# GlaireDaggers/Pretty-Fast-Video

Measured on AMD Instinct MI355X. Metric: macroblocks/s (encode+decode) 1080p YUV420, higher is better.
Workload: dtype i32 (encoder transforms evaluated in exact f32; decoders i32)

## Files before the change

include/pfv_hip_ext.h:

```cpp
#ifndef PFV_HIP_EXT_H
#define PFV_HIP_EXT_H

#include "pfv_hip_core.h"

#ifdef __cplusplus
extern "C" {
#endif

PFV_API int pfv_ctx_create_prio(int device, int priority, pfv_ctx **out);
PFV_API int pfv_ctx_pci_bus_id(pfv_ctx *ctx, char *out, int len);
PFV_API int pfv_device_sync(pfv_ctx *ctx);
PFV_API void *pfv_ctx_stream(pfv_ctx *ctx);

typedef enum pfv_option {
    PFV_OPT_ENC_TRANSFORM = 1, PFV_OPT_TILE_COMPACTION = 2, PFV_OPT_LANE_MAPPING = 3, PFV_OPT_ENTROPY_DECODE = 4,
    PFV_OPT_ENTDEC_LANE_BITS = 5, PFV_OPT_ENTDEC_LAUNCHES = 6, PFV_OPT_ENTDEC_INNER_ROUNDS = 7
} pfv_option;
enum { PFV_ENTROPY_DECODE_AUTO = 0, PFV_ENTROPY_DECODE_HOST = 1, PFV_ENTROPY_DECODE_DEVICE = 2 };
enum { PFV_LANES_AUTO = 0, PFV_LANES_PER_MB_8 = 1, PFV_LANES_PER_MB_16 = 2 };
enum { PFV_ENC_TRANSFORM_AUTO = 0, PFV_ENC_TRANSFORM_INT = 1 };
PFV_API int pfv_ctx_set_option(pfv_ctx *ctx, int option, int value);
PFV_API int pfv_ctx_get_option(pfv_ctx *ctx, int option, int *value);

typedef struct pfv_event pfv_event;
PFV_API int pfv_event_create(pfv_ctx *ctx, pfv_event **out);
PFV_API int pfv_event_record(pfv_event *e);
PFV_API int pfv_event_elapsed_ms(pfv_event *start, pfv_event *stop, float *ms);
PFV_API void pfv_event_destroy(pfv_event *e);
PFV_API int pfv_ctx_wait_event(pfv_ctx *ctx, pfv_event *e);

typedef struct pfv_graph pfv_graph;
PFV_API int pfv_graph_begin(pfv_ctx *ctx);
PFV_API int pfv_graph_end(pfv_ctx *ctx, pfv_graph **out);
PFV_API int pfv_graph_launch(pfv_graph *g);
PFV_API void pfv_graph_destroy(pfv_graph *g);

PFV_API int pfv_blit_dev(pfv_ctx *ctx, uint8_t *dst, int dst_w, int dst_h, const uint8_t *src, int src_w, int src_h,
                         int dx, int dy, int sx, int sy, int sw, int sh);

PFV_API int pfv_reduce_dev(pfv_ctx *ctx, uint8_t *dst, const uint8_t *src, int src_w, int src_h);
PFV_API int pfv_double_dev(pfv_ctx *ctx, uint8_t *dst, const uint8_t *src, int src_w, int src_h);
PFV_API int pfv_rgb_to_yuv420_dev(pfv_ctx *ctx, const uint8_t *rgb_dev, int width, int height, uint8_t *frame_dev);
PFV_API int pfv_yuv420_to_rgb_dev(pfv_ctx *ctx, const uint8_t *frame_dev, int width, int height, uint8_t *rgb_dev);

typedef struct pfv_comm pfv_comm;
enum { PFV_COMM_SUM = 0, PFV_COMM_MAX = 1 };
PFV_API int pfv_comm_unique_id(uint8_t id_out[128]);
PFV_API int pfv_comm_init(pfv_ctx *ctx, int rank, int world, const uint8_t id[128], pfv_comm **out);
PFV_API int pfv_comm_rank(const pfv_comm *c);
PFV_API int pfv_comm_world(const pfv_comm *c);
PFV_API int pfv_comm_broadcast_dev(pfv_comm *c, void *buf_dev, size_t bytes, int root);
PFV_API int pfv_comm_allreduce_f64_dev(pfv_comm *c, double *buf_dev, size_t count, int op);
PFV_API int pfv_comm_allgather_dev(pfv_comm *c, const void *send_dev, void *recv_dev, size_t bytes_per_rank);
PFV_API int pfv_comm_allreduce_f64(pfv_comm *c, double *values, size_t count, int op);
PFV_API int pfv_comm_barrier(pfv_comm *c);
PFV_API void pfv_comm_destroy(pfv_comm *c);

PFV_API int pfv_synth_frames_dev(pfv_ctx *ctx, int width, int height, int n_streams, const uint64_t *seeds, int t,
                                 uint8_t *frames_dev);
enum { PFV_SYNTH_PAN = 0, PFV_SYNTH_LOW_MOTION = 1, PFV_SYNTH_STATIC = 2 };
PFV_API int pfv_synth_frames_kind_dev(pfv_ctx *ctx, int width, int height, int n_streams, const uint64_t *seeds, int t, int kind,
                                      uint8_t *frames_dev);

PFV_API int pfv_dev_alloc(pfv_ctx *ctx, size_t bytes, void **out);
PFV_API int pfv_dev_free(pfv_ctx *ctx, void *p);
PFV_API int pfv_dev_copy(pfv_ctx *ctx, void *dst_dev, const void *src_dev, size_t bytes);
PFV_API int pfv_host_alloc(pfv_ctx *ctx, size_t bytes, void **out);
PFV_API int pfv_host_free(pfv_ctx *ctx, void *p);
PFV_API int pfv_dev_upload(pfv_ctx *ctx, void *dst_dev, const void *src_host, size_t bytes);
// ... 145 lines not shown
```

pretty-fast-video_amd/_lib.py:

```python
from __future__ import annotations

import ctypes
import os
from ctypes import POINTER, c_char_p, c_float, c_int, c_size_t, c_uint8, c_void_p

_HERE = os.path.dirname(os.path.abspath(__file__))
DEFAULT_LIB = os.path.join(_HERE, "libpfv_hip.so")

PFV_OK = 0
PFV_ERR_BAD_ARG = -1
PFV_ERR_HIP = -2
PFV_ERR_NOMEM = -3
PFV_ERR_BAD_MV = -4
PFV_ERR_NO_DEVICE = -5
PFV_ERR_FORMAT = -6
PFV_ERR_VERSION = -7
PFV_ERR_IO = -8
PFV_ERR_STATE = -9

PFV_COMM_SUM, PFV_COMM_MAX = 0, 1
PFV_OPT_ENC_TRANSFORM = 1
PFV_OPT_TILE_COMPACTION = 2
PFV_OPT_LANE_MAPPING = 3
PFV_LANES_AUTO, PFV_LANES_PER_MB_8, PFV_LANES_PER_MB_16 = 0, 1, 2
PFV_OPT_ENTROPY_DECODE = 4
PFV_OPT_ENTDEC_LANE_BITS, PFV_OPT_ENTDEC_LAUNCHES, PFV_OPT_ENTDEC_INNER_ROUNDS = 5, 6, 7
PFV_ENTROPY_DECODE_AUTO, PFV_ENTROPY_DECODE_HOST, PFV_ENTROPY_DECODE_DEVICE = 0, 1, 2
PFV_ENC_TRANSFORM_AUTO, PFV_ENC_TRANSFORM_INT = 0, 1
PFV_FRAME_PACKED, PFV_FRAME_PADDED = 0, 1


class PfvError(RuntimeError):
    def __init__(self, code: int, msg: str):
        super().__init__(f"pfv_hip error {code}: {msg}")
        self.code = code


_P = c_void_p
SIGNATURES = [
    ("pfv_device_count", c_int, []),
    ("pfv_ctx_create", c_int, [c_int, POINTER(_P)]),
    ("pfv_ctx_create_prio", c_int, [c_int, c_int, POINTER(_P)]),
    ("pfv_ctx_destroy", None, [_P]),
    ("pfv_ctx_pci_bus_id", c_int, [_P, _P, c_int]),
    ("pfv_ctx_sync", c_int, [_P]),
    ("pfv_device_sync", c_int, [_P]),
    ("pfv_ctx_stream", _P, [_P]),
    ("pfv_last_error", c_char_p, [_P]),
    ("pfv_version", c_char_p, []),
    ("pfv_ctx_set_option", c_int, [_P, c_int, c_int]),
    ("pfv_ctx_get_option", c_int, [_P, c_int, POINTER(c_int)]),
    ("pfv_event_create", c_int, [_P, POINTER(_P)]),
    ("pfv_event_record", c_int, [_P]),
    ("pfv_event_elapsed_ms", c_int, [_P, _P, POINTER(c_float)]),
    ("pfv_event_destroy", None, [_P]),
    ("pfv_ctx_wait_event", c_int, [_P, _P]),
    ("pfv_graph_begin", c_int, [_P]),
    ("pfv_graph_end", c_int, [_P, POINTER(_P)]),
    ("pfv_graph_launch", c_int, [_P]),
    ("pfv_graph_destroy", None, [_P]),
    ("pfv_pad16", c_int, [c_int]),
    ("pfv_qtables_from_quality", c_int, [c_int, _P, _P, _P, _P, POINTER(c_float)]),
    ("pfv_encode_plane", c_int, [_P, _P, c_int, c_int, _P, c_uint8, _P]),
    ("pfv_encode_plane_delta", c_int, [_P, _P, c_int, c_int, _P, _P, c_float, c_uint8, _P, _P, _P]),
    ("pfv_decode_plane_into", c_int, [_P, _P, c_int, c_int, _P, _P]),
    ("pfv_decode_plane_delta", c_int, [_P, _P, _P, _P, c_int, c_int, _P, _P, _P]),
    ("pfv_decode_plane_delta_into", c_int, [_P, _P, _P, _P, c_int, c_int, _P, _P]),
    ("pfv_blit_dev", c_int, [_P, _P, c_int, c_int, _P, c_int, c_int, c_int, c_int, c_int, c_int, c_int, c_int]),
    ("pfv_reduce_dev", c_int, [_P, _P, _P, c_int, c_int]),
    ("pfv_double_dev", c_int, [_P, _P, _P, c_int, c_int]),
    ("pfv_rgb_to_yuv420_dev", c_int, [_P, _P, c_int, c_int, _P]),
    ("pfv_yuv420_to_rgb_dev", c_int, [_P, _P, c_int, c_int, _P]),
    ("pfv_comm_unique_id", c_int, [_P]),
    ("pfv_comm_init", c_int, [_P, c_int, c_int, _P, POINTER(_P)]),
    ("pfv_comm_rank", c_int, [_P]),
    ("pfv_comm_world", c_int, [_P]),
    ("pfv_comm_broadcast_dev", c_int, [_P, _P, c_size_t, c_int]),
    ("pfv_comm_allreduce_f64_dev", c_int, [_P, _P, c_size_t, c_int]),
    ("pfv_comm_allgather_dev", c_int, [_P, _P, _P, c_size_t]),
# ... 172 lines not shown
```

pretty-fast-video_amd/csrc/pfv_context.hip:

```cpp
struct pfv_ctx {
    int device = 0;
    hipStream_t stream = nullptr;
    std::string err;
    void *scratch[8] = {};
    size_t scratch_cap[8] = {};
    QTab *qtab_dev = nullptr;
    QTab *qtab_host = nullptr;
    int *flag_dev = nullptr;
    int n_cus = 256;
    bool capturing = false;
    int opt_enc_transform = PFV_ENC_TRANSFORM_AUTO;
    int opt_tile_compaction = 1;
    int opt_lane_mapping = PFV_LANES_AUTO;
    int opt_entropy_decode = PFV_ENTROPY_DECODE_AUTO;
    int opt_entdec_lane_bits = (int)kEdSubBits, opt_entdec_launches = 3, opt_entdec_inner = kEdInner;
    std::vector<struct pfv_comm *> comms;
    std::mutex comms_m;
    pfv_ctx *owner = nullptr;
    std::vector<pfv_ctx *> children;
    int priority = 0;
};
static int ctx_create_child(pfv_ctx *user, pfv_ctx **out)
{
    int rc = pfv_ctx_create_prio(user->device, user->priority, out);
    if (rc) return rc;
    (*out)->owner = user;
    std::lock_guard<std::mutex> lk(user->comms_m);
    user->children.push_back(*out);
    return PFV_OK;
}
static void comm_teardown(struct pfv_comm *c);

static thread_local std::string g_tls_err;

static int fail(pfv_ctx *ctx, int code, const std::string &msg)
{
    if (ctx) ctx->err = msg;
    if (ctx && ctx->owner) ctx->owner->err = msg;
    g_tls_err = msg;
    return code;
}
static int hip_fail(pfv_ctx *ctx, hipError_t e, const char *what)
{
    (void)hipGetLastError();
    return fail(ctx, e == hipErrorOutOfMemory ? PFV_ERR_NOMEM : PFV_ERR_HIP,
                std::string(what) + ": " + hipGetErrorString(e));
}
#define HIP_TRY(ctx, expr)                                        \
    do {                                                          \
        hipError_t e__ = (expr);                                  \
        if (e__ != hipSuccess) return hip_fail(ctx, e__, #expr);  \
    } while (0)

static inline int pad16(int x) { return x + (16 - (x % 16)) % 16; }

extern "C" {

#ifndef PFV_BUILD_ID
#define PFV_BUILD_ID "unstamped"
#endif
PFV_API const char *pfv_version(void) { return "pfv-hip 0.2 (gfx950; pfv-rs 0.2.2 / codec 2.1.1 hot path; src " PFV_BUILD_ID ")"; }
PFV_API int pfv_pad16(int x) { return pad16(x); }

PFV_API const char *pfv_last_error(pfv_ctx *ctx) { return ctx ? ctx->err.c_str() : g_tls_err.c_str(); }

PFV_API int pfv_ctx_set_option(pfv_ctx *ctx, int option, int value)
{
    if (!ctx) return fail(nullptr, PFV_ERR_BAD_ARG, "null ctx");
    switch (option) {
    case PFV_OPT_ENC_TRANSFORM:
        if (value != PFV_ENC_TRANSFORM_AUTO && value != PFV_ENC_TRANSFORM_INT) return fail(ctx, PFV_ERR_BAD_ARG, "PFV_OPT_ENC_TRANSFORM: unknown value");
        ctx->opt_enc_transform = value;
        return PFV_OK;
    case PFV_OPT_TILE_COMPACTION:
        if (value < 0 || value > 2) return fail(ctx, PFV_ERR_BAD_ARG, "PFV_OPT_TILE_COMPACTION: 0, 1 or 2");
        ctx->opt_tile_compaction = value;
        return PFV_OK;
    case PFV_OPT_LANE_MAPPING:
        if (value != PFV_LANES_AUTO && value != PFV_LANES_PER_MB_8 && value != PFV_LANES_PER_MB_16) return fail(ctx, PFV_ERR_BAD_ARG, "PFV_OPT_LANE_MAPPING: unknown value");
        ctx->opt_lane_mapping = value;
        return PFV_OK;
    case PFV_OPT_ENTROPY_DECODE:
        if (value != PFV_ENTROPY_DECODE_AUTO && value != PFV_ENTROPY_DECODE_HOST && value != PFV_ENTROPY_DECODE_DEVICE) return fail(ctx, PFV_ERR_BAD_ARG, "PFV_OPT_ENTROPY_DECODE: unknown value");
        ctx->opt_entropy_decode = value;
        return PFV_OK;
    case PFV_OPT_ENTDEC_LANE_BITS:
        if (value < 32 || value > (int)kEdMaxSubBits || value % 32) return fail(ctx, PFV_ERR_BAD_ARG, "PFV_OPT_ENTDEC_LANE_BITS: a multiple of 32 in 32..256");
        ctx->opt_entdec_lane_bits = value;
        return PFV_OK;
    case PFV_OPT_ENTDEC_LAUNCHES:
        if (value < 1 || value > 64) return fail(ctx, PFV_ERR_BAD_ARG, "PFV_OPT_ENTDEC_LAUNCHES: 1..64");
        ctx->opt_entdec_launches = value;
        return PFV_OK;
    case PFV_OPT_ENTDEC_INNER_ROUNDS:
        if (value < 1 || value > 1024) return fail(ctx, PFV_ERR_BAD_ARG, "PFV_OPT_ENTDEC_INNER_ROUNDS: 1..1024");
        ctx->opt_entdec_inner = value;
        return PFV_OK;
    default:
        return fail(ctx, PFV_ERR_BAD_ARG, "pfv_ctx_set_option: unknown option");
    }
}
PFV_API int pfv_ctx_get_option(pfv_ctx *ctx, int option, int *value)
{
    if (!ctx || !value) return fail(ctx, PFV_ERR_BAD_ARG, "pfv_ctx_get_option: bad argument");
    switch (option) {
    case PFV_OPT_ENC_TRANSFORM: *value = ctx->opt_enc_transform; return PFV_OK;
    case PFV_OPT_TILE_COMPACTION: *value = ctx->opt_tile_compaction; return PFV_OK;
    case PFV_OPT_LANE_MAPPING: *value = ctx->opt_lane_mapping; return PFV_OK;
    case PFV_OPT_ENTROPY_DECODE: *value = ctx->opt_entropy_decode; return PFV_OK;
    case PFV_OPT_ENTDEC_LANE_BITS: *value = ctx->opt_entdec_lane_bits; return PFV_OK;
    case PFV_OPT_ENTDEC_LAUNCHES: *value = ctx->opt_entdec_launches; return PFV_OK;
    case PFV_OPT_ENTDEC_INNER_ROUNDS: *value = ctx->opt_entdec_inner; return PFV_OK;
    default: return fail(ctx, PFV_ERR_BAD_ARG, "pfv_ctx_get_option: unknown option");
    }
}

PFV_API int pfv_device_count(void)
{
    int n = 0;
    if (hipGetDeviceCount(&n) != hipSuccess) { (void)hipGetLastError(); return 0; }
    return n;
}

PFV_API int pfv_ctx_create(int device, pfv_ctx **out) { return pfv_ctx_create_prio(device, 0, out); }

PFV_API int pfv_ctx_create_prio(int device, int priority, pfv_ctx **out)
{
    if (!out) return fail(nullptr, PFV_ERR_BAD_ARG, "pfv_ctx_create: out is null");
    *out = nullptr;
    int n = 0;
    hipError_t e = hipGetDeviceCount(&n);
    if (e != hipSuccess || n <= 0) {
        (void)hipGetLastError();
        return fail(nullptr, PFV_ERR_NO_DEVICE, "pfv_ctx_create: no HIP device visible (the HIP path has no CPU fallback)");
    }
    if (device < 0 || device >= n) return fail(nullptr, PFV_ERR_BAD_ARG, "pfv_ctx_create: device ordinal out of range");
    HIP_TRY(nullptr, hipSetDevice(device));
    pfv_ctx *ctx = new pfv_ctx();
    ctx->device = device;
    ctx->priority = priority;
    {
        int cus = 0;
        if (hipDeviceGetAttribute(&cus, hipDeviceAttributeMultiprocessorCount, device) == hipSuccess && cus > 0) ctx->n_cus = cus;
    }
    if (priority == 0) {
        e = hipStreamCreateWithFlags(&ctx->stream, hipStreamNonBlocking);
    } else {
        int least = 0, greatest = 0;
        e = hipDeviceGetStreamPriorityRange(&least, &greatest);
        if (e == hipSuccess) e = hipStreamCreateWithPriority(&ctx->stream, hipStreamNonBlocking, priority > 0 ? greatest : least);
    }
    if (e == hipSuccess) e = hipMalloc((void **)&ctx->qtab_dev, 4 * sizeof(QTab));
    if (e == hipSuccess) e = hipHostMalloc((void **)&ctx->qtab_host, 4 * sizeof(QTab), hipHostMallocDefault);
    if (e == hipSuccess) e = hipMalloc((void **)&ctx->flag_dev, sizeof(int));
    if (e == hipSuccess) e = hipMemsetAsync(ctx->flag_dev, 0, sizeof(int), ctx->stream);
    if (e != hipSuccess) {
        int rc = hip_fail(nullptr, e, "pfv_ctx_create");
        pfv_ctx_destroy(ctx);
        return rc;
    }
    *out = ctx;
    return PFV_OK;
}

PFV_API void pfv_ctx_destroy(pfv_ctx *ctx)
// ... 160 lines not shown
```

pretty-fast-video_amd/csrc/pfv_device.h:

```cpp
#pragma once
#include <stdint.h>

#ifdef PFV_HIPEMU
#define PFV_WAVES_PER_EU(n)
#else
#define PFV_WAVES_PER_EU(n) __attribute__((amdgpu_waves_per_eu(n, n)))
#endif

namespace pfv {

constexpr int kStripMB = 8;
#ifndef PFV_STRIPS_PER_WG
#define PFV_STRIPS_PER_WG 4
#endif
constexpr int kStripsPerWG = PFV_STRIPS_PER_WG;
constexpr int kThreads = 64 * kStripsPerWG;

struct QTab {
    float rcp[64];
    int32_t deq[64];
};

struct PlaneGeom {
    int w, h;
    int pw, ph;
    int bw, bh;
    int strips_x;
    int strip0;
    int tiles_y;
    int tile0;
    int mb0;
    int qsel;
    int clear;
    int fast_src;
    long src_off;
    long pad_off;
};

struct FrameGeom {
    PlaneGeom p[3];
    int n_planes;
    int strips_per_frame;
    int tiles_per_frame;
    int mbs_per_frame;
    int n_streams;
    long src_frame_bytes;
    long pad_frame_bytes;
    const uint8_t *const *src_slots;
};
__host__ __device__ inline const uint8_t *frame_src(const FrameGeom &g, const uint8_t *src, int stream)
{
    return g.src_slots ? g.src_slots[stream] : src + (long)stream * g.src_frame_bytes;
}

struct CoefLists {
    const uint32_t *const *entries;
    const uint32_t *counts;
};
constexpr uint32_t coef_entry(uint32_t mb, uint32_t pos, int16_t value) { return ((uint32_t)(uint16_t)value << 16) | ((mb & 255u) << 8) | (pos & 255u); }

}
```

pretty-fast-video_amd/csrc/pfv_gop.hip:

```cpp
#pragma once

struct GopClock {
    std::chrono::steady_clock::time_point t0 = std::chrono::steady_clock::now();
    double lap()
    {
        const auto t1 = std::chrono::steady_clock::now();
        const double s = std::chrono::duration<double>(t1 - t0).count();
        t0 = t1;
        return s;
    }
};

struct GopTrace {
    bool on = getenv("PFV_GOP_TRACE") != nullptr;
    std::chrono::steady_clock::time_point t0 = std::chrono::steady_clock::now();
    void operator()(const char *what, long a = 0, long b = 0) const
    {
        if (on) fprintf(stderr, "[pfv gop %9.3f ms] %s %ld %ld\n", std::chrono::duration<double>(std::chrono::steady_clock::now() - t0).count() * 1e3, what, a, b);
    }
};

struct GopPacket {
    uint8_t type;
    int slot, t;
// ... 29 lines not shown
};

struct pfv_gop_encoder {
    pfv_ctx *ctx = nullptr;
    pfv_enc_session *hot = nullptr;
    int width = 0, height = 0, max_gops = 0, max_len = 0;
    size_t frame_bytes = 0, total_blocks = 0, arena_cap = 0;
    bool explicit_budget = false;
    int quality = 0;
    long batches_redone = 0;
    std::vector<uint32_t> redo_sizes;
    GopEncBatch batch[2];
    int cur = 0;
    hipStream_t copy_stream = nullptr;
    hipStream_t down_stream = nullptr;
    int16_t *coef = nullptr;
    int8_t *mv = nullptr;
    uint8_t *has = nullptr;
    bool cont_valid = false;
    int cont_buf = 0, cont_slot = 0;
    PinnedBuf<EntEntry> entries_host;
    unsigned long long *cursor_host = nullptr;
    std::vector<uint8_t> out, drained;
    std::vector<pfv_iovec> segs, segs_drained;
    unsigned segs_in = 0;
    bool finished = false, failed = false;
    bool frames_by_ref = false;
    long frames_in = 0, batches = 0, frames_by_reference = 0;
    double stats[5] = {0, 0, 0, 0, 0};
    GopTrace trace;
};

template <class F>
static void gop_runs(const std::vector<int> &key, F &&fn)
{
    const int n = (int)key.size();
    for (int a = 0; a < n;) {
        if (key[(size_t)a] < 0) { a++; continue; }
        int b = a + 1;
        while (b < n && key[(size_t)b] == key[(size_t)a]) b++;
        fn(a, b - a, key[(size_t)a]);
        a = b;
    }
}

static void gop_enc_take_options(pfv_gop_encoder *e)
{
    pfv_ctx *k = e->ctx;
    const pfv_ctx *u = e->ctx->owner;
    if (!u) return;
    k->opt_enc_transform = u->opt_enc_transform;
    k->opt_tile_compaction = u->opt_tile_compaction;
    k->opt_lane_mapping = u->opt_lane_mapping;
}

static int gop_enc_submit(pfv_gop_encoder *e, GopEncBatch &B)
{
    pfv_ctx *ctx = e->ctx;
    pfv_enc_session *s = e->hot;
    const int G = (int)B.len.size();
    if (G == 0 || B.in_flight) return PFV_OK;
    GopClock clk;
    e->trace("submit begin: batch, groups", (long)(&B - e->batch), G);
    gop_enc_take_options(e);
    HIP_TRY(ctx, hipEventRecord(B.ev_uploaded, e->copy_stream));
    HIP_TRY(ctx, hipStreamWaitEvent(ctx->stream, B.ev_uploaded, 0));
    if (B.dev_frames) {
        if (!ctx->owner) return fail(ctx, PFV_ERR_STATE, "the context the encoder was created on has been destroyed: its device-frame copies have no stream");
        HIP_TRY(ctx, hipEventRecord(B.ev_dev_frames, ctx->owner->stream));
        HIP_TRY(ctx, hipStreamWaitEvent(ctx->stream, B.ev_dev_frames, 0));
    }
    const size_t pad = (size_t)s->geom.pad_frame_bytes;
    B.cont_saved = false;
    if (B.first_type[0] == 2 && e->cont_valid) {
        const uint8_t *src = s->prev[e->cont_buf] + (size_t)e->cont_slot * pad;
        uint8_t *dst = s->prev[s->cur];
        if (src != dst) HIP_TRY(ctx, hipMemcpyAsync(dst, src, pad, hipMemcpyDeviceToDevice, ctx->stream));
        if (!e->explicit_budget) {
            if (!B.cont_save) HIP_TRY(ctx, hipMalloc((void **)&B.cont_save, pad));
            HIP_TRY(ctx, hipMemcpyAsync(B.cont_save, src, pad, hipMemcpyDeviceToDevice, ctx->stream));
            B.cont_saved = true;
        }
    }
    HIP_TRY(ctx, hipMemsetAsync(B.cursor_dev, 0, sizeof(unsigned long long), ctx->stream));
    if (B.by_ref)
        HIP_TRY(ctx, hipMemcpyAsync(B.slots_dev, B.slots_host.data(), (size_t)e->max_len * (size_t)e->max_gops * sizeof(const uint8_t *), hipMemcpyHostToDevice, ctx->stream));
    int steps = 0;
    for (int l : B.len) steps = std::max(steps, l);
    const int cur0 = s->cur;
    std::vector<int> key((size_t)G);
    EntFrame f{};
    f.cap_bytes = s->ent_cap;
    for (int t = 0; t < steps; t++) {
        for (int k = 0; k < G; k++) key[(size_t)k] = B.len[(size_t)k] > t ? (t == 0 ? B.first_type[(size_t)k] : 2) : -1;
        const uint8_t *frames_t = B.frames_dev + (size_t)t * (size_t)e->max_gops * e->frame_bytes;
        int rc = PFV_OK;
        gop_runs(key, [&](int first, int count, int type) {
            if (!rc) rc = enc_launch(s, type == 2, first, count, frames_t, e->mv, e->has, e->coef, B.by_ref ? B.slots_dev + (size_t)t * (size_t)e->max_gops : nullptr);
            if (!rc) rc = ent_pack_win(s, type == 2, first, count, e->mv, e->has, e->coef);
            if (rc) return;
            EntEntry *ent = B.entries_dev + (size_t)t * (size_t)e->max_gops + (size_t)first;
            EntBufs b = s->ent;
            b.sizes += first;
            b.payload += (size_t)first * (size_t)s->ent_cap;
            hipLaunchKernelGGL(k_ent_retain, dim3(1), dim3(64), 0, ctx->stream, b.sizes, count, B.cursor_dev, (unsigned long long)B.arena_cap, ent, B.cursor_steps.data() + t);
            f.n_streams = count;
// ... 438 lines not shown
```

pretty-fast-video_amd/csrc/pfv_kernels.hip:

```cpp
#include <hip/hip_runtime.h>
#include <stdint.h>

#include "pfv_device.h"
#include "pfv_prof.h"


namespace pfv {

namespace {
__constant__ int kScale[64] = {
    32, 37, 34, 26, 32, 26, 34, 37, 37, 43, 39, 31, 37, 31, 39, 43, 34, 39, 35, 28, 34, 28, 35, 39, 26, 31, 28, 22, 26, 22,
    28, 31, 32, 37, 34, 26, 32, 26, 34, 37, 26, 31, 28, 22, 26, 22, 28, 31, 34, 39, 35, 28, 34, 28, 35, 39, 37, 43, 39, 31,
    37, 31, 39, 43,
};
__constant__ int kInvZigzag[64] = {
    0,  1,  5,  6,  14, 15, 27, 28, 2,  4,  7,  13, 16, 26, 29, 42, 3,  8,  12, 17, 25, 30, 41, 43, 9,  11, 18, 24, 31, 40,
    44, 53, 10, 19, 23, 32, 39, 45, 52, 54, 20, 22, 33, 38, 46, 51, 55, 60, 21, 34, 37, 47, 50, 56, 59, 61, 35, 36, 48, 49,
    57, 58, 62, 63,
};
}

constexpr int kWinRows = 16 * kStripsPerWG + 30;
constexpr int kWinStride = 176;
constexpr int kWinBytes = kWinRows * kWinStride;
// ... 26 lines not shown
        unsigned b = (unsigned)v >> 31;
        h = (int)((unsigned)v + b) >> 1;
        q = (int)((unsigned)h + b) >> 1;
    }
};
struct TDiv416 {
    int x, q, s;
    __host__ __device__ __forceinline__ explicit TDiv416(int v) : x(v)
    {
        unsigned b = (unsigned)(v >> 31) & 3u;
        q = (int)((unsigned)v + b) >> 2;
        s = (int)((unsigned)q + b) >> 2;
    }
};
__host__ __device__ __forceinline__ int tdiv2(int x) { return (int)((unsigned)x + ((unsigned)x >> 31)) >> 1; }

__device__ __forceinline__ void wave_lds_sync()
{
    __builtin_amdgcn_fence(__ATOMIC_RELEASE, "wavefront");
    __builtin_amdgcn_wave_barrier();
    __builtin_amdgcn_fence(__ATOMIC_ACQUIRE, "wavefront");
}

template <int CTRL>
__device__ __forceinline__ int dpp(int v)
{
    return __builtin_amdgcn_update_dpp(0, v, CTRL, 0xf, 0xf, true);
}
constexpr int kQuadXor1 = 0xB1;
constexpr int kQuadXor2 = 0x4E;
constexpr int kRowHalfMirror = 0x141;

__device__ __forceinline__ int mb_sum(int v)
{
    v += dpp<kQuadXor1>(v);
    v += dpp<kQuadXor2>(v);
    v += dpp<kRowHalfMirror>(v);
    return v;
}

__device__ __forceinline__ int xcd_remap(int b, int nb)
{
    int xcd = b & 7, idx = b >> 3;
    int per = nb >> 3, rem = nb & 7;
    return xcd * per + min(xcd, rem) + idx;
}

struct StripPos {
    int stream, plane;
    int sx, by;
    int x0, y0;
    int n_mb;
    int mb_first;
};

__device__ __forceinline__ int plane_of(const FrameGeom &g, int idx, bool tiles)
{
    int s1 = tiles ? g.p[1].tile0 : g.p[1].strip0, s2 = tiles ? g.p[2].tile0 : g.p[2].strip0;
    return (g.n_planes > 2 && idx >= s2) ? 2 : ((g.n_planes > 1 && idx >= s1) ? 1 : 0);
}
__device__ __forceinline__ void finish_strip(const FrameGeom &g, StripPos &s)
{
    const PlaneGeom &p = g.p[s.plane];
    s.x0 = s.sx * (kStripMB * 16);
    s.y0 = s.by * 16;
    s.n_mb = min(kStripMB, p.bw - s.sx * kStripMB);
    s.mb_first = p.mb0 + s.by * p.bw + s.sx * kStripMB;
}
__device__ __forceinline__ StripPos locate_strip(const FrameGeom &g, int gstrip)
{
    StripPos s;
    s.stream = gstrip / g.strips_per_frame;
    int st = gstrip - s.stream * g.strips_per_frame;
    s.plane = plane_of(g, st, false);
    const PlaneGeom &p = g.p[s.plane];
    st -= p.strip0;
    s.by = st / p.strips_x;
    s.sx = st - s.by * p.strips_x;
    finish_strip(g, s);
    return s;
}

__host__ __device__ __forceinline__ void fdct8(int (&v)[8])
{
    int a0 = wadd(v[0], v[7]), a1 = wadd(v[1], v[6]), a2 = wadd(v[2], v[5]), a3 = wadd(v[3], v[4]);
    int a4 = wsub(v[0], v[7]), a5 = wsub(v[1], v[6]), a6 = wsub(v[2], v[5]), a7 = wsub(v[3], v[4]);
    int b0 = wadd(a0, a3), b1 = wadd(a1, a2), b2 = wsub(a0, a3), b3 = wsub(a1, a2);
    int c0 = wadd(b0, b1), c1 = wsub(b0, b1);
    int c2 = wadd(wadd(b2, b2 >> 2), b3 >> 1);
    int c3 = wsub(wsub(b2 >> 1, b3), b3 >> 2);
    int a4q = a4 >> 2, a7q = a7 >> 2;
    int b4 = wsub(wadd(wadd(a7q, a4), a4q), a4 >> 4);
    int b7 = wadd(wsub(wsub(a4q, a7), a7q), a7 >> 4);
    int b5 = wsub(wsub(wadd(a5, a6), a6 >> 2), a6 >> 4);
    int b6 = wadd(wadd(wsub(a6, a5), a5 >> 2), a5 >> 4);
    int c4 = wadd(b4, b5), c5 = wsub(b4, b5), c6 = wadd(b6, b7), c7 = wsub(b6, b7);
    v[0] = c0; v[1] = c4; v[2] = c2; v[3] = wsub(c5, c7);
    v[4] = c1; v[5] = wadd(c5, c7); v[6] = c3; v[7] = c6;
}

__host__ __device__ __forceinline__ void idct8(int (&v)[8])
{
    int c0 = v[0], d4 = v[1], d6 = v[3], c1 = v[4], d5 = v[5], d7 = v[7];
    TDiv24 c2(v[2]), c3(v[6]);
    int c4 = d4, c5 = wadd(d5, d6), c7 = wsub(d5, d6), c6 = d7;
    TDiv416 b4(wadd(c4, c5)), b5(wsub(c4, c5)), b6(wadd(c6, c7)), b7(wsub(c6, c7));
    int b0 = wadd(c0, c1), b1 = wsub(c0, c1);
    int b2 = wadd(wadd(c2.x, c2.q), c3.h);
    int b3 = wsub(wsub(c2.h, c3.x), c3.q);
    int a4 = wsub(wadd(wadd(b7.q, b4.x), b4.q), b4.s);
    int a7 = wadd(wsub(wsub(b4.q, b7.x), b7.q), b7.s);
    int a5 = wadd(wadd(wsub(b5.x, b6.x), b6.q), b6.s);
    int a6 = wsub(wsub(wadd(b6.x, b5.x), b5.q), b5.s);
    int a0 = wadd(b0, b2), a1 = wadd(b1, b3), a2 = wsub(b1, b3), a3 = wsub(b0, b2);
    v[0] = wadd(a0, a4); v[1] = wadd(a1, a5); v[2] = wadd(a2, a6); v[3] = wadd(a3, a7);
    v[4] = wsub(a3, a7); v[5] = wsub(a2, a6); v[6] = wsub(a1, a5); v[7] = wsub(a0, a4);
}

__device__ __forceinline__ void rows_to_cols2(int (&v)[2][8], int *mb, int i, int mx)
{
// ... 39 lines not shown
    __device__ __forceinline__ float rcp(int k) const { return __int_as_float(tab[(k * 8 + c) * 4 + 0]); }
    __device__ __forceinline__ int scale(int k) const { return tab[(k * 8 + c) * 4 + 1]; }
    __device__ __forceinline__ int zz(int k) const { return tab[(k * 8 + c) * 4 + 2]; }
    __device__ __forceinline__ int deq(int k) const { return tab[(k * 8 + c) * 4 + 3]; }
    __device__ __forceinline__ float deqf(int k) const { return __int_as_float(tab[(k * 8 + c) * 4 + 3]); }
};
constexpr int kQTabDwords = 4 * 64;
template <bool ENC, bool FLT = false>
__device__ __forceinline__ int4 load_qentry(const QTab *qt, int lane)
{
    int4 e;
    e.x = ENC ? __float_as_int(qt->rcp[lane]) : 0;
    e.y = ENC ? (FLT ? (kScale[lane] << 16) : kScale[lane]) : 0;
    e.z = kInvZigzag[lane];
    e.w = FLT ? __float_as_int((float)qt->deq[lane]) : qt->deq[lane];
    return e;
}
template <bool ENC, bool FLT = false>
__device__ __forceinline__ void fill_qtable(int *tab, const QTab *qt, int lane)
{
    reinterpret_cast<int4 *>(tab)[lane] = load_qentry<ENC, FLT>(qt, lane);
}
__device__ __forceinline__ unsigned pack4(int a, int b, int c, int d)
{
    return (unsigned)a | ((unsigned)b << 8) | ((unsigned)c << 16) | ((unsigned)d << 24);
}
__device__ __forceinline__ int byte_of(unsigned w, int i) { return (int)((w >> (8 * i)) & 0xffu); }

__device__ __forceinline__ void unpack_row(const uint4 &row, int (&px)[2][8])
{
#pragma unroll
    for (int k = 0; k < 4; k++) {
        px[0][k] = byte_of(row.x, k); px[0][k + 4] = byte_of(row.y, k);
        px[1][k] = byte_of(row.z, k); px[1][k + 4] = byte_of(row.w, k);
    }
}
__device__ __forceinline__ uint4 pack_row(const int (&px)[2][8])
{
    return make_uint4(pack4(px[0][0], px[0][1], px[0][2], px[0][3]), pack4(px[0][4], px[0][5], px[0][6], px[0][7]),
                      pack4(px[1][0], px[1][1], px[1][2], px[1][3]), pack4(px[1][4], px[1][5], px[1][6], px[1][7]));
}

__device__ __forceinline__ uint4 ld_stream(const uint4 *p)
{
    return make_uint4(__builtin_nontemporal_load(&p->x), __builtin_nontemporal_load(&p->y), __builtin_nontemporal_load(&p->z),
                      __builtin_nontemporal_load(&p->w));
}
__device__ __forceinline__ void st_stream(uint4 *p, const uint4 &v)
{
    __builtin_nontemporal_store(v.x, &p->x); __builtin_nontemporal_store(v.y, &p->y);
    __builtin_nontemporal_store(v.z, &p->z); __builtin_nontemporal_store(v.w, &p->w);
}

__device__ __forceinline__ uint4 load_src16(const uint8_t *plane, const PlaneGeom &p, int x, int y)
{
    unsigned fill = (unsigned)p.clear * 0x01010101u;
    uint4 val = make_uint4(fill, fill, fill, fill);
    if (y < p.h && x < p.w) {
        const uint8_t *src = plane + (long)y * p.w + x;
        if (p.fast_src && x + 16 <= p.w) {
            val = *reinterpret_cast<const uint4 *>(src);
        } else {
            unsigned wds[4];
#pragma unroll
            for (int i = 0; i < 4; i++) {
                unsigned acc = 0;
#pragma unroll
                for (int b = 0; b < 4; b++) {
                    int xx = x + i * 4 + b;
                    unsigned px = xx < p.w ? (unsigned)src[i * 4 + b] : (unsigned)p.clear;
                    acc |= px << (8 * b);
                }
                wds[i] = acc;
            }
            val = make_uint4(wds[0], wds[1], wds[2], wds[3]);
        }
    }
    return val;
}

__device__ __forceinline__ uint4 load_unaligned16(const uint8_t *p)
{
    int sh = (int)((uintptr_t)p & 3);
    const unsigned *d = reinterpret_cast<const unsigned *>(p - sh);
    unsigned d0 = d[0], d1 = d[1], d2 = d[2], d3 = d[3], d4 = sh ? d[4] : 0u;
    return make_uint4(__builtin_amdgcn_alignbyte(d1, d0, sh), __builtin_amdgcn_alignbyte(d2, d1, sh),
                      __builtin_amdgcn_alignbyte(d3, d2, sh), __builtin_amdgcn_alignbyte(d4, d3, sh));
}

__device__ __forceinline__ void store_cropped16(uint8_t *plane, const PlaneGeom &p, int x, int y, const uint4 &val)
{
    if (y < p.h && x < p.w) st_stream(reinterpret_cast<uint4 *>(plane + (long)y * p.w + x), val);
}

typedef __attribute__((address_space(3))) void lds_void_t;
typedef __attribute__((address_space(1))) const void gbl_cvoid_t;

__device__ __forceinline__ int stage_chunk(int ch) { return (ch >> 4) * kStageChunks + (ch & 15); }
__device__ __forceinline__ void store_coef_half(const int *stage, int16_t *coef_mb0, int n_mb, int lane, int h)
{
#pragma unroll
    for (int j = 0; j < 2; j++) {
        int ch = j * 64 + lane;
        int mb = ch >> 4;
        if (mb < n_mb) st_stream(&reinterpret_cast<uint4 *>(coef_mb0)[mb * 32 + h * 16 + (ch & 15)], reinterpret_cast<const uint4 *>(stage)[stage_chunk(ch)]);
    }
}
__device__ __forceinline__ void fetch_coef_half(uint4 (&buf)[2], const int16_t *coef_mb0, int n_mb, int lane, int h)
{
#pragma unroll
    for (int j = 0; j < 2; j++) {
        int ch = j * 64 + lane;
        int mb = ch >> 4;
        buf[j] = make_uint4(0, 0, 0, 0);
        if (mb < n_mb) buf[j] = ld_stream(&reinterpret_cast<const uint4 *>(coef_mb0)[mb * 32 + h * 16 + (ch & 15)]);
    }
}
__device__ __forceinline__ void store_coef_quads(const int *stage, int16_t *coef_mb0, int n_mb, int lane, int half_strip)
{
#pragma unroll
    for (int j = 0; j < 2; j++) {
        int ch = j * 64 + lane;
        int mb = half_strip * 4 + (ch >> 5);
        if (mb < n_mb) st_stream(&reinterpret_cast<uint4 *>(coef_mb0)[half_strip * 128 + ch], reinterpret_cast<const uint4 *>(stage)[stage_chunk(ch)]);
    }
}
__device__ __forceinline__ void fetch_coef_quads(uint4 (&buf)[2], const int16_t *coef_mb0, int n_mb, int lane, int half_strip)
{
#pragma unroll
    for (int j = 0; j < 2; j++) {
        int ch = j * 64 + lane;
        int mb = half_strip * 4 + (ch >> 5);
        buf[j] = make_uint4(0, 0, 0, 0);
        if (mb < n_mb) buf[j] = ld_stream(&reinterpret_cast<const uint4 *>(coef_mb0)[half_strip * 128 + ch]);
    }
}
__device__ __forceinline__ void stage_coef_half(int *stage, const uint4 (&buf)[2], int lane)
{
#pragma unroll
    for (int j = 0; j < 2; j++) reinterpret_cast<uint4 *>(stage)[stage_chunk(j * 64 + lane)] = buf[j];
}

struct ListSpan {
    const uint32_t *ent;
    uint32_t lo, hi;
    uint32_t e0, e1;
};
__device__ __forceinline__ ListSpan list_span(const uint32_t *ent, uint32_t begin, uint32_t end, int last_lane, int lane)
{
    ListSpan sp{ent, 0u, 0u, 0u, 0u};
    sp.lo = (uint32_t)__builtin_amdgcn_readlane((int)begin, 0);
    sp.hi = (uint32_t)__builtin_amdgcn_readlane((int)end, last_lane);
    if (sp.hi < sp.lo) sp.hi = sp.lo;
    const uint32_t k = sp.lo + (uint32_t)lane;
    if (k < sp.hi) sp.e0 = ent[k];
    if (k + 64u < sp.hi) sp.e1 = ent[k + 64u];
    return sp;
}
template <int LPM>
__device__ __forceinline__ void stage_list_put(int16_t *stage, uint32_t e, int mb_low, int h)
{
    const int pos = (int)(e & 255u), mbl = (int)(((e >> 8) - (uint32_t)mb_low) & 255u);
    if (LPM == 8) {
        if ((pos >> 7) == h && mbl < kStripMB) stage[mbl * (2 * kStagePitch) + (pos & 127)] = (int16_t)(e >> 16);
    } else {
        if (mbl < kStripMB / 2) stage[(mbl * 2 + (pos >> 7)) * (2 * kStagePitch) + (pos & 127)] = (int16_t)(e >> 16);
    }
}
template <int LPM>
// ... 166 lines not shown
    return f2{__builtin_fmaf(r[0], 256.0f, -256.0f * kQuantMagic), __builtin_fmaf(r[1], 256.0f, -256.0f * kQuantMagic)};
}
__device__ __forceinline__ int16_t quant_low16(float biased) { return (int16_t)__float_as_int(biased); }
__device__ __forceinline__ void forward_half_f(f2 (&x)[8], int *xw, int m, int i, const LaneQ &lq, float magic)
{
    int *mb = xw + m * kMBPitch;
    ffdct8(x);
    f_rows_to_cols(x, mb, i, m & 3);
    ffdct8(x);
    int16_t *stage = reinterpret_cast<int16_t *>(xw) + m * (2 * kStagePitch);
#pragma unroll
    for (int k = 0; k < 8; k++) {
        const int zz = lq.zz(k);
        f2 biased;
        x[k] = quant_pair_f(x[k], lq.scale(k), lq.rcp(k), magic, biased);
#pragma unroll
        for (int s = 0; s < 2; s++) stage[s * 64 + zz] = quant_low16(biased[s]);
    }
    wave_lds_sync();
}
constexpr float kPixelBias = 127.501953125f;
__device__ __forceinline__ f2 iframe_pixel_f(f2 x) { return x * f2s(1.0f / 256.0f) + f2s(kPixelBias); }
template <bool PIXEL>
__device__ __forceinline__ void inverse_half_f(f2 (&c)[8], int *xw, int m, int i, const LaneQ &lq)
{
    int *mb = xw + m * kMBPitch;
#pragma unroll
    for (int k = 0; k < 8; k++) c[k] = c[k] * f2s(lq.deqf(k));
    fidct8(c);
    f_cols_to_rows(c, mb, i, m & 3);
    fidct8(c);
#pragma unroll
    for (int k = 0; k < 8; k++) c[k] = PIXEL ? iframe_pixel_f(c[k]) : f2floor(c[k] * f2s(1.0f / 256.0f));
}
__device__ __forceinline__ uint4 pack_row_f(const f2 (&px)[8])
{
    unsigned w[4] = {0, 0, 0, 0};
#pragma unroll
    for (int k = 0; k < 8; k++) {
        w[k >> 2] = __builtin_amdgcn_cvt_pk_u8_f32(px[k][0], (unsigned)(k & 3), w[k >> 2]);
        w[2 + (k >> 2)] = __builtin_amdgcn_cvt_pk_u8_f32(px[k][1], (unsigned)(k & 3), w[2 + (k >> 2)]);
    }
    return make_uint4(w[0], w[1], w[2], w[3]);
}
__device__ __forceinline__ void unpack_row_f(const uint4 &row, f2 (&px)[8])
{
#pragma unroll
    for (int k = 0; k < 4; k++) {
        px[k] = f2{(float)byte_of(row.x, k), (float)byte_of(row.z, k)};
        px[k + 4] = f2{(float)byte_of(row.y, k), (float)byte_of(row.w, k)};
    }
}

template <bool FLT, int LPM = 8>
__global__ __launch_bounds__(kThreads) void k_enc_iframe(FrameGeom g, const uint8_t *__restrict__ src,
                                                          int16_t *__restrict__ coef, uint8_t *__restrict__ recon,
                                                          const QTab *__restrict__ qtabs, float qmagic)
{
    __shared__ __attribute__((aligned(16))) int xchg[kStripsPerWG][kXchgDwords];
    __shared__ __attribute__((aligned(16))) int qtab_lds[kStripsPerWG][kQTabDwords];
    constexpr int kPasses = LPM == 8 ? 2 : 1;

    const int lane = threadIdx.x & 63, wave = __builtin_amdgcn_readfirstlane((int)(threadIdx.x >> 6));
    const int gw = xcd_remap((int)blockIdx.x, (int)gridDim.x) * kStripsPerWG + wave;
    const int gstrip = LPM == 8 ? gw : gw >> 1, half_strip = LPM == 8 ? 0 : gw & 1;
    if (gstrip >= g.strips_per_frame * g.n_streams) return;
    const StripPos sp = locate_strip(g, gstrip);
    if (half_strip * 4 >= sp.n_mb) return;
    const PlaneGeom &p = g.p[sp.plane];
    const int slot = lane >> 3, i = lane & 7;
    const int m = LPM == 8 ? slot : half_strip * 4 + (slot >> 1);
    int *xw = xchg[wave];

    fill_qtable<true, FLT>(qtab_lds[wave], qtabs + p.qsel, lane);
    const uint8_t *plane = frame_src(g, src, sp.stream) + p.src_off;
    uint4 rows[kPasses];
#pragma unroll
    for (int pass = 0; pass < kPasses; pass++) rows[pass] = load_src16(plane, p, sp.x0 + m * 16, sp.y0 + i + 8 * (LPM == 8 ? pass : (slot & 1)));

    wave_lds_sync();
    const LaneQ lq{qtab_lds[wave], i};
    int16_t *coef_mb0 = coef + ((long)sp.stream * g.mbs_per_frame + sp.mb_first) * 256;
    uint8_t *dst = recon ? recon + (long)sp.stream * g.pad_frame_bytes + p.pad_off + (long)(sp.y0 + i) * p.pw + sp.x0 + m * 16
                         : nullptr;
#pragma unroll
    for (int pass = 0; pass < kPasses; pass++) {
        const int h = LPM == 8 ? pass : (slot & 1);
        if (FLT) {
            f2 x[8];
            unpack_row_f(rows[pass], x);
#pragma unroll
            for (int k = 0; k < 8; k++) x[k] = x[k] * f2s(256.0f) - f2s(32768.0f);
            forward_half_f(x, xw, slot, i, lq, qmagic);
            if (LPM == 8) store_coef_half(xw, coef_mb0, sp.n_mb, lane, h);
            else store_coef_quads(xw, coef_mb0, sp.n_mb, lane, half_strip);
            wave_lds_sync();
            if (recon) {
                inverse_half_f<true>(x, xw, slot, i, lq);
                if (m < sp.n_mb) *reinterpret_cast<uint4 *>(dst + (long)(8 * h) * p.pw) = pack_row_f(x);
            }
        } else {
            int v[2][8];
            unpack_row(rows[pass], v);
#pragma unroll
            for (int s = 0; s < 2; s++) {
#pragma unroll
                for (int k = 0; k < 8; k++) v[s][k] = (int)((unsigned)(v[s][k] - 128) << 8);
            }
            forward_half(v, xw, slot, i, lq, true);
            if (LPM == 8) store_coef_half(xw, coef_mb0, sp.n_mb, lane, h);
            else store_coef_quads(xw, coef_mb0, sp.n_mb, lane, half_strip);
            wave_lds_sync();
            if (recon) {
                inverse_half(v, xw, slot, i, lq);
#pragma unroll
                for (int s = 0; s < 2; s++)
#pragma unroll
                    for (int k = 0; k < 8; k++) v[s][k] = min(max(v[s][k] + 128, 0), 255);
                if (m < sp.n_mb) *reinterpret_cast<uint4 *>(dst + (long)(8 * h) * p.pw) = pack_row(v);
            }
        }
    }
}

struct SearchState {
    int cx, cy;
    int err;
};

__device__ __forceinline__ unsigned dot_ab(const uint4 &a, unsigned b0, unsigned b1, unsigned b2, unsigned b3, unsigned acc)
{
    acc = __builtin_amdgcn_udot4(a.x, b0, acc, false);
    acc = __builtin_amdgcn_udot4(a.y, b1, acc, false);
    acc = __builtin_amdgcn_udot4(a.z, b2, acc, false);
    return __builtin_amdgcn_udot4(a.w, b3, acc, false);
}
__device__ __forceinline__ unsigned sq2(unsigned x, unsigned y, unsigned acc)
{
    return __builtin_amdgcn_udot4(y, y, __builtin_amdgcn_udot4(x, x, acc, false), false);
}
__device__ __forceinline__ unsigned sq4(unsigned b0, unsigned b1, unsigned b2, unsigned b3, unsigned acc) { return sq2(b2, b3, sq2(b0, b1, acc)); }

constexpr int kPencSplit = -1;
constexpr int kPsWaves = 7;
constexpr int kTfWaves = 7;
constexpr int kPencCompactMax = 16;
constexpr int kRedPitch = 72;
constexpr int kRedDwords = kStripMB * kRedPitch;
struct SearchLane {
    int neg2;
    int ord;
    int dy, dx;
    int *wr;
    const int4 *rd;
};
__device__ __forceinline__ SearchLane make_search_lane(int *red, int m, int i, int neg2)
{
    SearchLane sl;
    sl.neg2 = neg2;
    sl.ord = i + 1;
    const int b9 = i < 4 ? i : i + 1;
    sl.dy = b9 / 3 - 1;
    sl.dx = b9 - (b9 / 3) * 3 - 1;
    sl.wr = red + m * kRedPitch + i;
    sl.rd = reinterpret_cast<const int4 *>(red + m * kRedPitch + i * 8);
    return sl;
}
__device__ __forceinline__ unsigned mb_min(unsigned v)
{
    v = min(v, (unsigned)dpp<kQuadXor1>((int)v));
    v = min(v, (unsigned)dpp<kQuadXor2>((int)v));
    v = min(v, (unsigned)dpp<kRowHalfMirror>((int)v));
    return v;
}
// ... 134 lines not shown
#pragma unroll
        for (int mx = -1; mx <= 1; mx++) {
            if (my == 0 && mx == 0) continue;
            sl.wr[ord * 8] = part[my + 1][mx + 1];
            ord++;
        }
    }
    wave_lds_sync();
    const int4 x = sl.rd[0], y = sl.rd[1];
    wave_lds_sync();
    err = a2 + ((x.x + x.y) + (x.z + x.w)) + ((y.x + y.y) + (y.z + y.w));
    }
    bool valid = true;
    if (BOUNDS) {
        const int oy = mby + st.cy + sl.dy * S, ox = mbx + st.cx + sl.dx * S;
        valid = oy >= 0 && oy <= ph - 16 && ox >= 0 && ox <= pw - 16;
    }
    const unsigned key = valid ? (((unsigned)err << 4) | (unsigned)sl.ord) : 0xffffffffu;
    const unsigned centre = FIRST ? ((unsigned)(a2 + mb_sum(part[1][1])) << 4) : ((unsigned)st.err << 4);
    const unsigned best = min(mb_min(key), centre);
    const int bo = (int)(best & 15u);
    st.err = (int)(best >> 4);
    st.cy += ((int)((0x2A501u >> (2 * bo)) & 3u) - 1) * S;
    st.cx += ((int)((0x24891u >> (2 * bo)) & 3u) - 1) * S;
}

#ifndef PFV_PENC_WAVES
#define PFV_PENC_WAVES 5
#endif
struct TilePos {
    StripPos sp;
    int plane_ty;
    int winx0, winy0;
    bool wave_valid;
};
__device__ __forceinline__ TilePos locate_tile(const FrameGeom &g, int vt, int wave)
{
    TilePos t;
    t.sp.stream = vt / g.tiles_per_frame;
    int tl = vt - t.sp.stream * g.tiles_per_frame;
    t.sp.plane = plane_of(g, tl, true);
    const PlaneGeom &p = g.p[t.sp.plane];
    tl -= p.tile0;
    t.plane_ty = tl / p.strips_x;
    t.sp.sx = tl - t.plane_ty * p.strips_x;
    t.sp.by = t.plane_ty * kStripsPerWG + wave;
    finish_strip(g, t.sp);
    t.wave_valid = t.sp.by < p.bh;
    t.winx0 = t.sp.x0 - 16;
    t.winy0 = t.plane_ty * (16 * kStripsPerWG) - 15;
    return t;
}

__device__ __forceinline__ void issue_window(const PlaneGeom &p, const uint8_t *refp, const TilePos &t, uint8_t *winbuf, int wave,
                                             int lane)
{
    const int q0 = win_first_issue(wave), q1 = win_first_issue(wave + 1);
#pragma unroll 5
    for (int q = q0; q < q1; q++) {
        const int c = q * 64 + lane;
        const int row = c / kWinChunksPerRow, col = c - row * kWinChunksPerRow;
        const int y = min(max(t.winy0 + row, 0), p.ph - 1), x = min(max(t.winx0 + col * 16, 0), p.pw - 16);
        __builtin_amdgcn_global_load_lds((gbl_cvoid_t *)(refp + (long)y * p.pw + x), (lds_void_t *)(winbuf + c * 16), 16, 0, 0);
    }
}

struct SearchOut {
    int cx, cy;
    bool coded;
    uint4 patch[2];
};

template <bool DPPRED = false>
__device__ __forceinline__ void penc_search(const FrameGeom &g, const TilePos &tp, const uint8_t *win, int *red, const uint4 (&rows)[2], int lane,
                                            float min_err, int neg2, SearchOut &so)
{
    const StripPos &sp = tp.sp;
    const PlaneGeom &p = g.p[sp.plane];
    const int m = lane >> 3, i = lane & 7;
    const bool mb_valid = m < sp.n_mb;
    const int mbx = sp.x0 + m * 16, mby = sp.y0;
    const int wcol0 = mbx - tp.winx0;
    const int wrow0 = mby - tp.winy0 + i;

    unsigned s2 = 0;
#pragma unroll
    for (int h = 0; h < 2; h++) {
        s2 = __builtin_amdgcn_udot4(rows[h].x, rows[h].x, s2, false);
        s2 = __builtin_amdgcn_udot4(rows[h].y, rows[h].y, s2, false);
        s2 = __builtin_amdgcn_udot4(rows[h].z, rows[h].z, s2, false);
        s2 = __builtin_amdgcn_udot4(rows[h].w, rows[h].w, s2, false);
    }
    const int a2 = mb_sum((int)s2);

    SearchState st;
    st.cx = 0; st.cy = 0; st.err = 0;
    const SearchLane sl = make_search_lane(red, m, i, neg2);
    const bool interior = sp.x0 >= 16 && sp.x0 + kStripMB * 16 + 16 <= p.pw && sp.y0 >= 16 && sp.y0 + 32 <= p.ph;
    if (interior) {
        search_level<8, true, false, DPPRED>(win, wrow0, wcol0, rows[0], rows[1], a2, mbx, mby, p.pw, p.ph, st, sl);
        KMARK(3);
        search_level<4, false, false, DPPRED>(win, wrow0, wcol0, rows[0], rows[1], a2, mbx, mby, p.pw, p.ph, st, sl);
        KMARK(4);
        search_level<2, false, false, DPPRED>(win, wrow0, wcol0, rows[0], rows[1], a2, mbx, mby, p.pw, p.ph, st, sl);
        KMARK(5);
        search_level<1, false, false, DPPRED>(win, wrow0, wcol0, rows[0], rows[1], a2, mbx, mby, p.pw, p.ph, st, sl);
        KMARK(6);
    } else {
        search_level<8, true, true, DPPRED>(win, wrow0, wcol0, rows[0], rows[1], a2, mbx, mby, p.pw, p.ph, st, sl);
        search_level<4, false, true, DPPRED>(win, wrow0, wcol0, rows[0], rows[1], a2, mbx, mby, p.pw, p.ph, st, sl);
        search_level<2, false, true, DPPRED>(win, wrow0, wcol0, rows[0], rows[1], a2, mbx, mby, p.pw, p.ph, st, sl);
        search_level<1, false, true, DPPRED>(win, wrow0, wcol0, rows[0], rows[1], a2, mbx, mby, p.pw, p.ph, st, sl);
    }

    so.coded = mb_valid && !((float)st.err <= min_err);
    so.cx = st.cx; so.cy = st.cy;

    const int wx = wcol0 + st.cx, shp = wx & 3;
    const uint8_t *rp = win + (wrow0 + st.cy) * kWinStride + (wx & ~3);
#pragma unroll
    for (int h = 0; h < 2; h++) {
        const unsigned *d = reinterpret_cast<const unsigned *>(rp + 8 * h * kWinStride);
        unsigned d0 = d[0], d1 = d[1], d2 = d[2], d3 = d[3], d4 = d[4];
        so.patch[h] = make_uint4(__builtin_amdgcn_alignbyte(d1, d0, shp), __builtin_amdgcn_alignbyte(d2, d1, shp),
                                 __builtin_amdgcn_alignbyte(d3, d2, shp), __builtin_amdgcn_alignbyte(d4, d3, shp));
    }
}

__device__ __forceinline__ void opaque_row(uint4 &r)
{
#ifndef PFV_HIPEMU
    asm volatile("" : "+v"(r.x), "+v"(r.y), "+v"(r.z), "+v"(r.w));
#else
    (void)r;
#endif
}
template <bool FLT, bool REUNPACK = false, class Store>
__device__ __forceinline__ uint4 penc_half(const uint4 &srow, const uint4 &prow, int *xw, int m, int i, const LaneQ &lq, float qmagic, bool want_recon,
                                           Store &&store)
{
    uint4 out = prow;
    if (FLT) {
        f2 x[8], pp[8];
        unpack_row_f(srow, x);
        unpack_row_f(prow, pp);
#pragma unroll
        for (int k = 0; k < 8; k++) x[k] = residual_f(x[k], pp[k]);
        forward_half_f(x, xw, m, i, lq, qmagic);
        store();
        wave_lds_sync();
        if (want_recon) {
            inverse_half_f<false>(x, xw, m, i, lq);
            if (REUNPACK) {
                uint4 again = prow;
                opaque_row(again);
                unpack_row_f(again, pp);
            }
#pragma unroll
            for (int k = 0; k < 8; k++) {
                const f2 t = f2{__builtin_fminf(x[k][0], 127.0f), __builtin_fminf(x[k][1], 127.0f)};
                pp[k] = pp[k] + t * f2s(2.0f);
            }
            out = pack_row_f(pp);
        }
    } else {
        int v[2][8], pp[2][8];
        unpack_row(srow, v);
        unpack_row(prow, pp);
#pragma unroll
        for (int s = 0; s < 2; s++) {
#pragma unroll
            for (int k = 0; k < 8; k++) {
                int d = v[s][k] - pp[s][k];
                v[s][k] = (int)((unsigned)tdiv2(d) << 8);
            }
        }
        forward_half(v, xw, m, i, lq, true);
        store();
        wave_lds_sync();
        if (want_recon) {
            inverse_half(v, xw, m, i, lq);
#pragma unroll
            for (int s = 0; s < 2; s++) {
#pragma unroll
                for (int k = 0; k < 8; k++)
                    pp[s][k] = min(max(pp[s][k] + 2 * v[s][k], 0), 255);
            }
            out = pack_row(pp);
        }
    }
    return out;
}

__device__ __forceinline__ void penc_store_skipped(int16_t *coef_mb, uint8_t *dst, long pw, int i, const uint4 (&patch)[2])
{
#pragma unroll
    for (int j = 0; j < 4; j++) st_stream(&reinterpret_cast<uint4 *>(coef_mb)[j * 8 + i], make_uint4(0, 0, 0, 0));
    if (dst) {
        *reinterpret_cast<uint4 *>(dst) = patch[0];
        *reinterpret_cast<uint4 *>(dst + 8 * pw) = patch[1];
    }
}

template <bool FLT>
__device__ __forceinline__ void penc_transform(const FrameGeom &g, const TilePos &tp, const SearchOut &so, const uint4 (&rows)[2], int *xw,
                                               int lane, int16_t *__restrict__ coef, uint8_t *__restrict__ recon, const int *qtab_lds, float qmagic)
{
    const StripPos &sp = tp.sp;
    const PlaneGeom &p = g.p[sp.plane];
    const int m = lane >> 3, i = lane & 7;
    const bool mb_valid = m < sp.n_mb, coded = so.coded;
    const int mbx = sp.x0 + m * 16;
    int16_t *coef_mb0 = coef + ((long)sp.stream * g.mbs_per_frame + sp.mb_first) * 256;
    uint8_t *dst = recon ? recon + (long)sp.stream * g.pad_frame_bytes + p.pad_off + (long)(sp.y0 + i) * p.pw + mbx : nullptr;

    if (__any(coded)) {
        const LaneQ lq{qtab_lds, i};
#pragma unroll
        for (int h = 0; h < 2; h++) {
            const uint4 o = penc_half<FLT>(coded ? rows[h] : so.patch[h], so.patch[h], xw, m, i, lq, qmagic, recon != nullptr,
                                           [&]() { store_coef_half(xw, coef_mb0, sp.n_mb, lane, h); });
            if (h == 0) KMARK(9);
            if (recon && mb_valid) *reinterpret_cast<uint4 *>(dst + (long)(8 * h) * p.pw) = o;
        }
    } else if (mb_valid) {
        penc_store_skipped(coef_mb0 + m * 256, dst, p.pw, i, so.patch);
    }
}

template <bool FLT>
__device__ __forceinline__ void penc_transform_compact(const FrameGeom &g, const TilePos &tp, int wave, int n_coded, const int *slot_orig,
                                                       const uint4 *staged, int *xw, int lane, int16_t *__restrict__ coef,
                                                       uint8_t *__restrict__ recon, const int *qtab_lds, float qmagic)
{
    const PlaneGeom &p = g.p[tp.sp.plane];
    const int m = lane >> 3, i = lane & 7;
    const int slot = wave * 8 + m;
    const bool has = slot < n_coded;
    const long tile_mb0 = (long)tp.sp.stream * g.mbs_per_frame + p.mb0 + (long)(tp.plane_ty * kStripsPerWG) * p.bw + tp.sp.sx * kStripMB;
    const LaneQ lq{qtab_lds, i};
    const uint4 *sl = staged + (has ? slot : 0) * 32 + i * 4;
#pragma unroll
    for (int h = 0; h < 2; h++) {
        uint4 srow = sl[h], prow = sl[2 + h];
        if (!has) srow = prow = make_uint4(0, 0, 0, 0);
        const uint4 o = penc_half<FLT>(srow, prow, xw, m, i, lq, qmagic, recon != nullptr, [&]() {
#pragma unroll
            for (int j = 0; j < 2; j++) {
                const int ch = j * 64 + lane, sc = wave * 8 + (ch >> 4);
                if (sc < n_coded) {
                    const int og = slot_orig[sc];
                    int16_t *mb = coef + (tile_mb0 + (long)(og >> 3) * p.bw + (og & 7)) * 256;
                    st_stream(&reinterpret_cast<uint4 *>(mb)[h * 16 + (ch & 15)], reinterpret_cast<const uint4 *>(xw)[stage_chunk(ch)]);
                }
            }
        });
        if (recon && has) {
            const int orig = slot_orig[slot];
            uint8_t *dst = recon + (long)tp.sp.stream * g.pad_frame_bytes + p.pad_off +
                           (long)((tp.plane_ty * kStripsPerWG + (orig >> 3)) * 16 + i + 8 * h) * p.pw + tp.sp.x0 + (orig & 7) * 16;
            *reinterpret_cast<uint4 *>(dst) = o;
        }
    }
}

template <bool FLT>
__global__ __launch_bounds__(kThreads) PFV_WAVES_PER_EU(PFV_PENC_WAVES) void k_enc_pframe(FrameGeom g, const uint8_t *__restrict__ src,
                                                          const uint8_t *__restrict__ ref, int8_t *__restrict__ mv_out,
                                                          uint8_t *__restrict__ has_out, int16_t *__restrict__ coef,
                                                          uint8_t *__restrict__ recon, const QTab *__restrict__ qtabs,
                                                          float min_err, int neg2, float qmagic, int compact_max)
{
    __shared__ __attribute__((aligned(16))) uint8_t win_lds[16 + kWinAlloc];
    __shared__ __attribute__((aligned(16))) int red_lds[kStripsPerWG][kRedDwords];
    __shared__ __attribute__((aligned(16))) int qtab_lds[kQTabDwords];
    uint8_t *win = win_lds + 16;

    const int lane = threadIdx.x & 63, wave = __builtin_amdgcn_readfirstlane((int)(threadIdx.x >> 6));
    const int m = lane >> 3, i = lane & 7;
    const int vt = xcd_remap((int)blockIdx.x, (int)gridDim.x);
    const TilePos cur = locate_tile(g, vt, wave);
    const PlaneGeom &p = g.p[cur.sp.plane];
    if (wave == 0) fill_qtable<true, FLT>(qtab_lds, qtabs + p.qsel, lane);

    KMARK(0);
    KMARK_WHERE();
    issue_window(p, ref + (long)cur.sp.stream * g.pad_frame_bytes + p.pad_off, cur, win, wave, lane);
    uint4 rows[2];
    rows[0] = rows[1] = make_uint4(0, 0, 0, 0);
    if (cur.wave_valid) {
        const uint8_t *plane = frame_src(g, src, cur.sp.stream) + p.src_off;
        rows[0] = load_src16(plane, p, cur.sp.x0 + m * 16, cur.sp.y0 + i);
        rows[1] = load_src16(plane, p, cur.sp.x0 + m * 16, cur.sp.y0 + i + 8);
    }
    KMARK(1);
    __syncthreads();
    KMARK(2);
    SearchOut so;
    so.cx = so.cy = 0; so.coded = false;
    so.patch[0] = so.patch[1] = make_uint4(0, 0, 0, 0);
    if (cur.wave_valid) penc_search(g, cur, win, red_lds[wave], rows, lane, min_err, neg2, so);
    KMARK(7);
    const bool mb_valid = cur.wave_valid && m < cur.sp.n_mb;
    if (i == 0 && mb_valid) {
        const long mbi = (long)cur.sp.stream * g.mbs_per_frame + cur.sp.mb_first + m;
        mv_out[mbi * 2 + 0] = (int8_t)so.cx;
        mv_out[mbi * 2 + 1] = (int8_t)so.cy;
        has_out[mbi] = so.coded ? 1 : 0;
    }
    constexpr int kMaskAt = (kStripsPerWG - 1) * kRedDwords + kRedDwords - 8;
    int *red_all = &red_lds[0][0];
    {
        const unsigned long long bal = __ballot(so.coded);
        unsigned mine = 0;
#pragma unroll
        for (int k = 0; k < kStripMB; k++) mine |= (unsigned)((bal >> (8 * k)) & 1ull) << k;
        if (lane == 0) red_all[kMaskAt + wave] = (int)mine;
    }
    __syncthreads();
    KMARK(8);
    unsigned tile_mask = 0;
#pragma unroll
    for (int k = 0; k < kStripsPerWG; k++) tile_mask |= (unsigned)__builtin_amdgcn_readfirstlane(red_all[kMaskAt + k]) << (8 * k);
    int n_coded = __builtin_popcount(tile_mask), strips_coded = 0;
#pragma unroll
    for (int k = 0; k < kStripsPerWG; k++) strips_coded += ((tile_mask >> (8 * k)) & 0xffu) ? 1 : 0;
    int *xw = reinterpret_cast<int *>(win + win_first_issue(wave) * 1024);
    constexpr int kCompactMax = kPencCompactMax;
    constexpr int kSlotOrigAt = kCompactMax * 128;
    static_assert(kSlotOrigAt + kCompactMax <= kMaskAt, "staging area + slot table must fit below the strip masks");
    static_assert(kStripsPerWG * 8 <= 32, "one bit per macroblock of the tile");
    if (n_coded <= compact_max && ((n_coded + 7) >> 3) < strips_coded) {
        uint4 *stage4 = reinterpret_cast<uint4 *>(red_all);
        const int place = wave * 8 + m;
        if (so.coded) {
            const int slot = __builtin_popcount(tile_mask & ((1u << place) - 1u));
            uint4 *sl = stage4 + slot * 32 + i * 4;
            sl[0] = rows[0]; sl[1] = rows[1]; sl[2] = so.patch[0]; sl[3] = so.patch[1];
            if (i == 0) red_all[kSlotOrigAt + slot] = place;
        } else if (mb_valid) {
            const PlaneGeom &pp = g.p[cur.sp.plane];
            penc_store_skipped(coef + ((long)cur.sp.stream * g.mbs_per_frame + cur.sp.mb_first + m) * 256,
                               recon ? recon + (long)cur.sp.stream * g.pad_frame_bytes + pp.pad_off + (long)(cur.sp.y0 + i) * pp.pw + cur.sp.x0 + m * 16 : nullptr,
                               pp.pw, i, so.patch);
        }
        __syncthreads();
        if (wave * 8 < n_coded)
            penc_transform_compact<FLT>(g, cur, wave, n_coded, red_all + kSlotOrigAt, stage4, xw, lane, coef, recon, qtab_lds, qmagic);
    } else if (cur.wave_valid) {
        penc_transform<FLT>(g, cur, so, rows, xw, lane, coef, recon, qtab_lds, qmagic);
    }
    KMARK(11);
}

template <bool DPPRED>
__global__ __launch_bounds__(kThreads) PFV_WAVES_PER_EU(kPsWaves) void k_pf_search(FrameGeom g, const uint8_t *__restrict__ src,
                                                          const uint8_t *__restrict__ ref, int8_t *__restrict__ mv_out,
                                                          uint8_t *__restrict__ has_out, int16_t *__restrict__ coef,
                                                          uint8_t *__restrict__ recon, float min_err, int neg2)
{
    __shared__ __attribute__((aligned(16))) uint8_t win_lds[16 + kWinAlloc];
    __shared__ __attribute__((aligned(16))) int red_lds[DPPRED ? 1 : kStripsPerWG][DPPRED ? 4 : kRedDwords];
    uint8_t *win = win_lds + 16;

    const int lane = threadIdx.x & 63, wave = __builtin_amdgcn_readfirstlane((int)(threadIdx.x >> 6));
    const int m = lane >> 3, i = lane & 7;
    const int vt = xcd_remap((int)blockIdx.x, (int)gridDim.x);
    const TilePos cur = locate_tile(g, vt, wave);
    const PlaneGeom &p = g.p[cur.sp.plane];
    issue_window(p, ref + (long)cur.sp.stream * g.pad_frame_bytes + p.pad_off, cur, win, wave, lane);
    uint4 rows[2];
    rows[0] = rows[1] = make_uint4(0, 0, 0, 0);
    if (cur.wave_valid) {
        const uint8_t *plane = frame_src(g, src, cur.sp.stream) + p.src_off;
        rows[0] = load_src16(plane, p, cur.sp.x0 + m * 16, cur.sp.y0 + i);
        rows[1] = load_src16(plane, p, cur.sp.x0 + m * 16, cur.sp.y0 + i + 8);
    }
    __syncthreads();
    if (!cur.wave_valid) return;
    SearchOut so;
    penc_search<DPPRED>(g, cur, win, red_lds[DPPRED ? 0 : wave], rows, lane, min_err, neg2, so);
    if (m < cur.sp.n_mb) {
        const long mbi = (long)cur.sp.stream * g.mbs_per_frame + cur.sp.mb_first + m;
        if (i == 0) {
            mv_out[mbi * 2 + 0] = (int8_t)so.cx;
            mv_out[mbi * 2 + 1] = (int8_t)so.cy;
            has_out[mbi] = so.coded ? 1 : 0;
        }
        if (!so.coded)
            penc_store_skipped(coef + mbi * 256, recon ? recon + (long)cur.sp.stream * g.pad_frame_bytes + p.pad_off + (long)(cur.sp.y0 + i) * p.pw + cur.sp.x0 + m * 16 : nullptr,
                               p.pw, i, so.patch);
    }
}

constexpr int kTfStrips = 8;
__host__ __device__ __forceinline__ int tf_groups_of_plane(const PlaneGeom &p) { return (p.strips_x * p.bh + kTfStrips - 1) / kTfStrips; }
__host__ __device__ __forceinline__ int tf_groups_per_frame(const FrameGeom &g)
{
    int n = 0;
    for (int k = 0; k < g.n_planes; k++) n += tf_groups_of_plane(g.p[k]);
    return n;
}

template <bool FLT>
__global__ __launch_bounds__(64) PFV_WAVES_PER_EU(kTfWaves) void k_pf_transform(FrameGeom g, const uint8_t *__restrict__ src, const uint8_t *__restrict__ ref,
// ... 254 lines not shown
    if (wave_valid) {
        const int mbx = cur.sp.x0 + m * 16, mby = cur.sp.y0;
        const int wcol0 = mbx - cur.winx0, wrow0 = mby - cur.winy0 + r;
        unsigned s2 = __builtin_amdgcn_udot4(row.w, row.w, __builtin_amdgcn_udot4(row.z, row.z, __builtin_amdgcn_udot4(row.y, row.y, __builtin_amdgcn_udot4(row.x, row.x, 0, false), false), false), false);
        const int a2 = mb_sum16((int)s2);
        SearchState st;
        st.cx = 0; st.cy = 0; st.err = 0;
        const SearchLane16 sl = make_search_lane16(red_lds[wave], mb, r, neg2);
        const int hx0 = cur.sp.x0 + half_strip * 64;
        const bool interior = hx0 >= 16 && hx0 + 64 + 16 <= p.pw && cur.sp.y0 >= 16 && cur.sp.y0 + 32 <= p.ph;
        if (interior) {
            search_level16<8, true, false>(win, wrow0, wcol0, row, a2, mbx, mby, p.pw, p.ph, st, sl);
            search_level16<4, false, false>(win, wrow0, wcol0, row, a2, mbx, mby, p.pw, p.ph, st, sl);
            search_level16<2, false, false>(win, wrow0, wcol0, row, a2, mbx, mby, p.pw, p.ph, st, sl);
            search_level16<1, false, false>(win, wrow0, wcol0, row, a2, mbx, mby, p.pw, p.ph, st, sl);
        } else {
            search_level16<8, true, true>(win, wrow0, wcol0, row, a2, mbx, mby, p.pw, p.ph, st, sl);
            search_level16<4, false, true>(win, wrow0, wcol0, row, a2, mbx, mby, p.pw, p.ph, st, sl);
            search_level16<2, false, true>(win, wrow0, wcol0, row, a2, mbx, mby, p.pw, p.ph, st, sl);
            search_level16<1, false, true>(win, wrow0, wcol0, row, a2, mbx, mby, p.pw, p.ph, st, sl);
        }
        coded = mb_valid && !((float)st.err <= min_err);
        cx = st.cx; cy = st.cy;
        const int wx = wcol0 + cx, shp = wx & 3;
        const unsigned *d = reinterpret_cast<const unsigned *>(win + (wrow0 + cy) * kWinStride + (wx & ~3));
        const unsigned d0 = d[0], d1 = d[1], d2 = d[2], d3 = d[3], d4 = d[4];
        patch = make_uint4(__builtin_amdgcn_alignbyte(d1, d0, shp), __builtin_amdgcn_alignbyte(d2, d1, shp), __builtin_amdgcn_alignbyte(d3, d2, shp),
                           __builtin_amdgcn_alignbyte(d4, d3, shp));
    }
    const long mbi = (long)cur.sp.stream * g.mbs_per_frame + cur.sp.mb_first + m;
    if (r == 0 && mb_valid) {
        mv_out[mbi * 2 + 0] = (int8_t)cx;
        mv_out[mbi * 2 + 1] = (int8_t)cy;
        has_out[mbi] = coded ? 1 : 0;
    }
    __syncthreads();
    if (!wave_valid) return;
    int *xw = wave < kStripsPerWG ? reinterpret_cast<int *>(win) + wave * kXchgDwords : &red_lds[0][0] + (wave - kStripsPerWG) * kXchgDwords;
    int16_t *coef_mb0 = coef + ((long)cur.sp.stream * g.mbs_per_frame + cur.sp.mb_first) * 256;
    uint8_t *dst = recon ? recon + (long)cur.sp.stream * g.pad_frame_bytes + p.pad_off + (long)(cur.sp.y0 + r) * p.pw + cur.sp.x0 + m * 16 : nullptr;
    if (__any(coded)) {
        const LaneQ lq{qtab_lds, i};
        const uint4 o = penc_half<FLT>(coded ? row : patch, patch, xw, slot, i, lq, qmagic, recon != nullptr,
                                       [&]() { store_coef_quads(xw, coef_mb0, cur.sp.n_mb, lane, half_strip); });
        if (recon && mb_valid) *reinterpret_cast<uint4 *>(dst) = o;
    } else if (mb_valid) {
        uint4 *cm = reinterpret_cast<uint4 *>(coef_mb0 + m * 256);
        st_stream(&cm[r], make_uint4(0, 0, 0, 0));
        st_stream(&cm[16 + r], make_uint4(0, 0, 0, 0));
        if (dst) *reinterpret_cast<uint4 *>(dst) = patch;
    }
}

template <int LPM = 8, bool LISTS = false>
__global__ __launch_bounds__(kThreads) void k_dec_iframe(FrameGeom g, const int16_t *__restrict__ coef, CoefLists cl,
                                                          uint8_t *__restrict__ out, const QTab *__restrict__ qtabs,
                                                          uint8_t *__restrict__ frames_out)
{
    __shared__ __attribute__((aligned(16))) int xchg[kStripsPerWG][kXchgDwords];
    __shared__ __attribute__((aligned(16))) int qtab_lds[kStripsPerWG][kQTabDwords];
    constexpr int kPasses = LPM == 8 ? 2 : 1;

    const int lane = threadIdx.x & 63, wave = __builtin_amdgcn_readfirstlane((int)(threadIdx.x >> 6));
    const int gw = xcd_remap((int)blockIdx.x, (int)gridDim.x) * kStripsPerWG + wave;
    const int gstrip = LPM == 8 ? gw : gw >> 1, half_strip = LPM == 8 ? 0 : gw & 1;
    if (gstrip >= g.strips_per_frame * g.n_streams) return;
    const StripPos sp = locate_strip(g, gstrip);
    if (half_strip * 4 >= sp.n_mb) return;
    const PlaneGeom &p = g.p[sp.plane];
    const int slot = lane >> 3, i = lane & 7;
    const int m = LPM == 8 ? slot : half_strip * 4 + (slot >> 1);
    int *xw = xchg[wave];

    const int16_t *coef_mb0 = coef + ((long)sp.stream * g.mbs_per_frame + sp.mb_first) * 256;
    uint4 cbuf[kPasses][2];
    ListSpan span;
    if (LISTS) {
        const int last = min(sp.n_mb - half_strip * 4, LPM == 8 ? 8 : 4) - 1;
        const uint32_t *cnt = cl.counts + (long)sp.stream * (g.mbs_per_frame + 1) + sp.mb_first + half_strip * 4;
        const int mw = min(LPM == 8 ? slot : (slot >> 1), last);
        span = list_span(cl.entries[sp.stream], cnt[mw], cnt[mw + 1], last * (LPM == 8 ? 8 : 16), lane);
    } else if (LPM == 8) {
        fetch_coef_half(cbuf[0], coef_mb0, sp.n_mb, lane, 0);
        fetch_coef_half(cbuf[kPasses - 1], coef_mb0, sp.n_mb, lane, 1);
    } else {
        fetch_coef_quads(cbuf[0], coef_mb0, sp.n_mb, lane, half_strip);
    }
    fill_qtable<false>(qtab_lds[wave], qtabs + p.qsel, lane);
    wave_lds_sync();
    const LaneQ lq{qtab_lds[wave], i};
    uint8_t *dst = out + (long)sp.stream * g.pad_frame_bytes + p.pad_off + (long)(sp.y0 + i) * p.pw + sp.x0 + m * 16;
#pragma unroll
    for (int pass = 0; pass < kPasses; pass++) {
        const int h = LPM == 8 ? pass : (slot & 1);
        if (LISTS) stage_list_half<LPM>(xw, span, lane, sp.mb_first + half_strip * 4, pass);
        else stage_coef_half(xw, cbuf[pass], lane);
        wave_lds_sync();
        int v[2][8];
        gather_half(v, xw, slot, lq);
        inverse_half(v, xw, slot, i, lq);
#pragma unroll
        for (int s = 0; s < 2; s++)
#pragma unroll
            for (int k = 0; k < 8; k++) v[s][k] = min(max(v[s][k] + 128, 0), 255);
        if (m < sp.n_mb) {
            const uint4 o = pack_row(v);
            *reinterpret_cast<uint4 *>(dst + (long)(8 * h) * p.pw) = o;
            if (frames_out)
                store_cropped16(frames_out + (long)sp.stream * g.src_frame_bytes + p.src_off, p, sp.x0 + m * 16, sp.y0 + i + 8 * h, o);
        }
    }
}

template <int LPM = 8, bool LISTS = false>
__global__ __launch_bounds__(kThreads) void k_dec_pframe(FrameGeom g, const int8_t *__restrict__ mv,
                                                          const uint8_t *__restrict__ has, const int16_t *__restrict__ coef, CoefLists cl,
                                                          const uint8_t *__restrict__ ref, uint8_t *__restrict__ out,
                                                          const QTab *__restrict__ qtabs, int *__restrict__ err_flag,
                                                          uint8_t *__restrict__ frames_out)
{
    __shared__ __attribute__((aligned(16))) int xchg[kStripsPerWG][kXchgDwords];
    __shared__ __attribute__((aligned(16))) int qtab_lds[kStripsPerWG][kQTabDwords];
    constexpr int kPasses = LPM == 8 ? 2 : 1;

    const int lane = threadIdx.x & 63, wave = __builtin_amdgcn_readfirstlane((int)(threadIdx.x >> 6));
    const int gw = xcd_remap((int)blockIdx.x, (int)gridDim.x) * kStripsPerWG + wave;
    const int gstrip = LPM == 8 ? gw : gw >> 1, half_strip = LPM == 8 ? 0 : gw & 1;
    if (gstrip >= g.strips_per_frame * g.n_streams) return;
    const StripPos sp = locate_strip(g, gstrip);
    if (half_strip * 4 >= sp.n_mb) return;
    const PlaneGeom &p = g.p[sp.plane];
    const int slot = lane >> 3, i = lane & 7;
    const int m = LPM == 8 ? slot : half_strip * 4 + (slot >> 1);
    int *xw = xchg[wave];
    const bool mb_valid = m < sp.n_mb;
    const long mbi = (long)sp.stream * g.mbs_per_frame + sp.mb_first + (mb_valid ? m : 0);

    int mx = mv[mbi * 2 + 0], my = mv[mbi * 2 + 1];
    const bool coded = mb_valid && has[mbi] != 0;
    uint32_t cnt0 = 0, cnt1 = 0;
    int last_mb = 0;
    if (LISTS) {
        last_mb = min(sp.n_mb - half_strip * 4, LPM == 8 ? 8 : 4) - 1;
        const uint32_t *cnt = cl.counts + (long)sp.stream * (g.mbs_per_frame + 1) + sp.mb_first + half_strip * 4;
        const int mw = min(LPM == 8 ? slot : (slot >> 1), last_mb);
        cnt0 = cnt[mw]; cnt1 = cnt[mw + 1];
    }
    fill_qtable<false>(qtab_lds[wave], qtabs + p.qsel, lane);

    const int mbx = sp.x0 + m * 16, mby = sp.y0;
    if (mb_valid) {
        int sx = mbx + mx, sy = mby + my;
        if (sx < 0 || sx > p.pw - 16 || sy < 0 || sy > p.ph - 16) {
            if (i == 0) atomicOr(err_flag + sp.stream, 1);
            mx = 0; my = 0;
        }
    }
    const bool any_coded = __any(coded);
    const int16_t *coef_mb0 = coef + ((long)sp.stream * g.mbs_per_frame + sp.mb_first) * 256;
    uint4 cbuf[kPasses][2];
    ListSpan span;
    if (any_coded) {
        if (LISTS) {
// ... 182 lines not shown
```

pretty-fast-video_amd/csrc/pfv_launch.hip:

```cpp
static float biased_rcp(int q)
{
    volatile float r = q ? 1.0f / (float)q : 0.0f;
    r = r * 1.000000476837158203125f;
    return r;
}
static int make_qtab(pfv_ctx *ctx, const int32_t q[64], QTab *out, bool decode_only = false)
{
    if (!q) return fail(ctx, PFV_ERR_BAD_ARG, "q-table is null");
    for (int i = 0; i < 64; i++)
        if (q[i] < (decode_only ? 0 : 1) || q[i] > 65535)
            return fail(ctx, PFV_ERR_BAD_ARG, decode_only ? "q-table entry outside [0,65535]" : "q-table entry outside [1,65535]");
    for (int i = 0; i < 64; i++) {
        out->rcp[i] = biased_rcp(q[i]);
        int z = H_INV_ZIGZAG[i];
        out->deq[i] = (int32_t)((uint32_t)H_SCALE[z] * (uint32_t)q[z]);
    }
    return PFV_OK;
}

static int ensure_scratch(pfv_ctx *ctx, int slot, size_t bytes, void **out)
{
    if (bytes == 0) bytes = 16;
    if (ctx->scratch_cap[slot] < bytes) {
        if (ctx->scratch[slot]) {
// ... 24 lines not shown
    p.fast_src = 0;
}

static FrameGeom plane_geom(int w, int h, int clear)
{
    FrameGeom g;
    memset(&g, 0, sizeof g);
    fill_plane(g.p[0], w, h, 0, 0, 0, 0, 0, clear);
    g.p[1] = g.p[0]; g.p[2] = g.p[0];
    g.n_planes = 1;
    g.strips_per_frame = g.p[0].strips_x * g.p[0].bh;
    g.tiles_per_frame = g.p[0].strips_x * g.p[0].tiles_y;
    g.mbs_per_frame = g.p[0].bw * g.p[0].bh;
    g.n_streams = 1;
    g.src_frame_bytes = (long)w * h;
    g.pad_frame_bytes = (long)g.p[0].pw * g.p[0].ph;
    g.p[0].fast_src = (w % 16 == 0);
    return g;
}

static FrameGeom frame_geom(int w, int h, int n_streams)
{
    FrameGeom g;
    memset(&g, 0, sizeof g);
    int cw = w / 2, ch = h / 2;
    fill_plane(g.p[0], w, h, 0, 0, 0, 0, 0, 0);
    long y_src = (long)w * h, y_pad = (long)g.p[0].pw * g.p[0].ph;
    int s1 = g.p[0].strips_x * g.p[0].bh, m1 = g.p[0].bw * g.p[0].bh;
    fill_plane(g.p[1], cw, ch, s1, m1, y_src, y_pad, 1, 128);
    long c_src = (long)cw * ch, c_pad = (long)g.p[1].pw * g.p[1].ph;
    int s2 = s1 + g.p[1].strips_x * g.p[1].bh, m2 = m1 + g.p[1].bw * g.p[1].bh;
    fill_plane(g.p[2], cw, ch, s2, m2, y_src + c_src, y_pad + c_pad, 1, 128);
    g.n_planes = 3;
    g.strips_per_frame = s2 + g.p[2].strips_x * g.p[2].bh;
    g.p[1].tile0 = g.p[0].strips_x * g.p[0].tiles_y;
    g.p[2].tile0 = g.p[1].tile0 + g.p[1].strips_x * g.p[1].tiles_y;
    g.tiles_per_frame = g.p[2].tile0 + g.p[2].strips_x * g.p[2].tiles_y;
    g.mbs_per_frame = m2 + g.p[2].bw * g.p[2].bh;
    g.n_streams = n_streams;
    g.src_frame_bytes = y_src + 2 * c_src;
    g.pad_frame_bytes = y_pad + 2 * c_pad;
    for (int i = 0; i < 3; i++)
        g.p[i].fast_src = (g.p[i].w % 16 == 0) && (g.p[i].src_off % 16 == 0) && (g.src_frame_bytes % 16 == 0);
    return g;
}

static FrameGeom with_base_alignment(FrameGeom g, const void *src_base)
{
    if (((uintptr_t)src_base & 15) != 0)
        for (int i = 0; i < 3; i++) g.p[i].fast_src = 0;
    return g;
}

static inline unsigned penc_blocks(const pfv_ctx *, const FrameGeom &g)
{
    return (unsigned)((long)g.tiles_per_frame * g.n_streams);
}

static inline unsigned strip_blocks(const FrameGeom &g)
{
    long strips = (long)g.strips_per_frame * g.n_streams;
    return (unsigned)((strips + kStripsPerWG - 1) / kStripsPerWG);
}

constexpr long kSmallGridStrips = 4096;
static inline bool use_small_grid(int opt, const FrameGeom &g)
{
    if (opt == PFV_LANES_PER_MB_8) return false;
    if (opt == PFV_LANES_PER_MB_16) return true;
    return (long)g.strips_per_frame * g.n_streams < kSmallGridStrips;
}
static inline unsigned half_strip_blocks(const FrameGeom &g)
{
    long waves = 2 * (long)g.strips_per_frame * g.n_streams;
    return (unsigned)((waves + kStripsPerWG - 1) / kStripsPerWG);
}
static void launch_enc_iframe(pfv_ctx *ctx, bool flt, bool small, const FrameGeom &g, const uint8_t *src, int16_t *coef, uint8_t *recon, const QTab *qt)
{
    if (small) {
        if (flt) hipLaunchKernelGGL((k_enc_iframe<true, 16>), dim3(half_strip_blocks(g)), dim3(kThreads), 0, ctx->stream, g, src, coef, recon, qt, kQuantMagic);
        else hipLaunchKernelGGL((k_enc_iframe<false, 16>), dim3(half_strip_blocks(g)), dim3(kThreads), 0, ctx->stream, g, src, coef, recon, qt, kQuantMagic);
    } else {
        if (flt) hipLaunchKernelGGL((k_enc_iframe<true, 8>), dim3(strip_blocks(g)), dim3(kThreads), 0, ctx->stream, g, src, coef, recon, qt, kQuantMagic);
        else hipLaunchKernelGGL((k_enc_iframe<false, 8>), dim3(strip_blocks(g)), dim3(kThreads), 0, ctx->stream, g, src, coef, recon, qt, kQuantMagic);
    }
}
static void launch_enc_pframe(pfv_ctx *ctx, bool flt, bool small, int compaction, const FrameGeom &g, const uint8_t *src, const uint8_t *ref, int8_t *mv,
                              uint8_t *has, int16_t *coef, uint8_t *recon, const QTab *qt, float min_err)
{
    const bool split = compaction == 2 && !small;
    launch_enc_pframe_kernels(ctx->stream, flt, small, split ? kPencSplit : (compaction ? kPencCompactMax : 0), g, penc_blocks(ctx, g), src, ref, mv, has, coef, recon, qt, min_err);
    if (split) {
        const unsigned tf = (unsigned)((long)g.n_streams * tf_groups_per_frame(g));
        if (flt) hipLaunchKernelGGL(k_pf_transform<true>, dim3(tf), dim3(64), 0, ctx->stream, g, src, ref, (const int8_t *)mv, (const uint8_t *)has, coef, recon, qt, kQuantMagic);
        else hipLaunchKernelGGL(k_pf_transform<false>, dim3(tf), dim3(64), 0, ctx->stream, g, src, ref, (const int8_t *)mv, (const uint8_t *)has, coef, recon, qt, kQuantMagic);
    }
}
struct DecCoefs {
    const int16_t *dense = nullptr;
    CoefLists lists{nullptr, nullptr};
    DecCoefs() = default;
    DecCoefs(const int16_t *d) : dense(d) {}
    DecCoefs(const uint32_t *const *entries, const uint32_t *counts) : lists{entries, counts} {}
    bool is_lists() const { return lists.entries != nullptr; }
    DecCoefs shifted(size_t slot, size_t mbs_per_frame) const
    {
        DecCoefs c;
        if (dense) c.dense = dense + slot * mbs_per_frame * 256;
        if (lists.entries) c.lists = CoefLists{lists.entries + slot, lists.counts + slot * (mbs_per_frame + 1)};
        return c;
    }
};
static void launch_dec_iframe(pfv_ctx *ctx, bool small, const FrameGeom &g, const DecCoefs &c, uint8_t *out, const QTab *qt, uint8_t *frames_out)
{
    const dim3 grid(small ? half_strip_blocks(g) : strip_blocks(g)), block(kThreads);
    if (c.is_lists()) {
        if (small) hipLaunchKernelGGL((k_dec_iframe<16, true>), grid, block, 0, ctx->stream, g, c.dense, c.lists, out, qt, frames_out);
        else hipLaunchKernelGGL((k_dec_iframe<8, true>), grid, block, 0, ctx->stream, g, c.dense, c.lists, out, qt, frames_out);
    } else {
        if (small) hipLaunchKernelGGL((k_dec_iframe<16, false>), grid, block, 0, ctx->stream, g, c.dense, c.lists, out, qt, frames_out);
        else hipLaunchKernelGGL((k_dec_iframe<8, false>), grid, block, 0, ctx->stream, g, c.dense, c.lists, out, qt, frames_out);
    }
}
static void launch_dec_pframe(pfv_ctx *ctx, bool small, const FrameGeom &g, const int8_t *mv, const uint8_t *has, const DecCoefs &c, const uint8_t *ref,
                              uint8_t *out, const QTab *qt, int *flag, uint8_t *frames_out)
{
    const dim3 grid(small ? half_strip_blocks(g) : strip_blocks(g)), block(kThreads);
    if (c.is_lists()) {
        if (small) hipLaunchKernelGGL((k_dec_pframe<16, true>), grid, block, 0, ctx->stream, g, mv, has, c.dense, c.lists, ref, out, qt, flag, frames_out);
        else hipLaunchKernelGGL((k_dec_pframe<8, true>), grid, block, 0, ctx->stream, g, mv, has, c.dense, c.lists, ref, out, qt, flag, frames_out);
    } else {
        if (small) hipLaunchKernelGGL((k_dec_pframe<16, false>), grid, block, 0, ctx->stream, g, mv, has, c.dense, c.lists, ref, out, qt, flag, frames_out);
        else hipLaunchKernelGGL((k_dec_pframe<8, false>), grid, block, 0, ctx->stream, g, mv, has, c.dense, c.lists, ref, out, qt, flag, frames_out);
    }
}

static int launch_check(pfv_ctx *ctx, const char *what)
{
    hipError_t e = hipGetLastError();
    if (e != hipSuccess) return hip_fail(ctx, e, what);
    return PFV_OK;
}

static int upload_qtabs(pfv_ctx *ctx, const int32_t *const *tables, int n, bool decode_only)
{
    for (int i = 0; i < n; i++) {
        int rc = make_qtab(ctx, tables[i], &ctx->qtab_host[i], decode_only);
        if (rc) return rc;
    }
    HIP_TRY(ctx, hipMemcpyAsync(ctx->qtab_dev, ctx->qtab_host, n * sizeof(QTab), hipMemcpyHostToDevice, ctx->stream));
    return PFV_OK;
}
```

pretty-fast-video_amd/csrc/pfv_plane_ops.hip:

```cpp
extern "C" {

PFV_API int pfv_encode_plane(pfv_ctx *ctx, const uint8_t *px, int w, int h, const int32_t q[64], uint8_t clear,
                             int16_t *coef_out)
{
    if (!ctx) return fail(nullptr, PFV_ERR_BAD_ARG, "null ctx");
    if (!px || !coef_out || w <= 0 || h <= 0) return fail(ctx, PFV_ERR_BAD_ARG, "pfv_encode_plane: bad argument");
    HIP_TRY(ctx, hipSetDevice(ctx->device));
    FrameGeom g = plane_geom(w, h, clear);
    const int32_t *tabs[1] = {q};
    int rc = upload_qtabs(ctx, tabs, 1, false);
    if (rc) return rc;
    void *d_src, *d_coef;
    size_t coef_bytes = (size_t)g.mbs_per_frame * 512;
    if ((rc = ensure_scratch(ctx, 0, (size_t)w * h, &d_src))) return rc;
    if ((rc = ensure_scratch(ctx, 1, coef_bytes, &d_coef))) return rc;
    HIP_TRY(ctx, hipMemcpyAsync(d_src, px, (size_t)w * h, hipMemcpyHostToDevice, ctx->stream));
    launch_enc_iframe(ctx, ctx->opt_enc_transform != PFV_ENC_TRANSFORM_INT, use_small_grid(ctx->opt_lane_mapping, g), g, (const uint8_t *)d_src, (int16_t *)d_coef,
                      nullptr, ctx->qtab_dev);
    if ((rc = launch_check(ctx, "k_enc_iframe"))) return rc;
    HIP_TRY(ctx, hipMemcpyAsync(coef_out, d_coef, coef_bytes, hipMemcpyDeviceToHost, ctx->stream));
    HIP_TRY(ctx, hipStreamSynchronize(ctx->stream));
    return PFV_OK;
}

PFV_API int pfv_encode_plane_delta(pfv_ctx *ctx, const uint8_t *px, int w, int h, const uint8_t *ref,
                                   const int32_t q[64], float px_err, uint8_t clear, int8_t *mv_out,
                                   uint8_t *has_coef_out, int16_t *coef_out)
{
    if (!ctx) return fail(nullptr, PFV_ERR_BAD_ARG, "null ctx");
    if (!px || !ref || !mv_out || !has_coef_out || !coef_out || w <= 0 || h <= 0)
        return fail(ctx, PFV_ERR_BAD_ARG, "pfv_encode_plane_delta: bad argument");
    HIP_TRY(ctx, hipSetDevice(ctx->device));
    FrameGeom g = plane_geom(w, h, clear);
    const int32_t *tabs[1] = {q};
    int rc = upload_qtabs(ctx, tabs, 1, false);
    if (rc) return rc;
    size_t n = (size_t)g.mbs_per_frame, coef_bytes = n * 512, pad_bytes = (size_t)g.pad_frame_bytes;
    void *d_src, *d_coef, *d_ref, *d_mv, *d_has;
    if ((rc = ensure_scratch(ctx, 0, (size_t)w * h, &d_src))) return rc;
    if ((rc = ensure_scratch(ctx, 1, coef_bytes, &d_coef))) return rc;
    if ((rc = ensure_scratch(ctx, 2, pad_bytes, &d_ref))) return rc;
    if ((rc = ensure_scratch(ctx, 3, n * 2, &d_mv))) return rc;
    if ((rc = ensure_scratch(ctx, 4, n, &d_has))) return rc;
    HIP_TRY(ctx, hipMemcpyAsync(d_src, px, (size_t)w * h, hipMemcpyHostToDevice, ctx->stream));
    HIP_TRY(ctx, hipMemcpyAsync(d_ref, ref, pad_bytes, hipMemcpyHostToDevice, ctx->stream));
    float min_err = px_err * px_err * 256.0f;
    launch_enc_pframe(ctx, ctx->opt_enc_transform != PFV_ENC_TRANSFORM_INT, use_small_grid(ctx->opt_lane_mapping, g), ctx->opt_tile_compaction, g,
                      (const uint8_t *)d_src, (const uint8_t *)d_ref, (int8_t *)d_mv, (uint8_t *)d_has, (int16_t *)d_coef, nullptr, ctx->qtab_dev, min_err);
    if ((rc = launch_check(ctx, "k_enc_pframe"))) return rc;
    HIP_TRY(ctx, hipMemcpyAsync(coef_out, d_coef, coef_bytes, hipMemcpyDeviceToHost, ctx->stream));
    HIP_TRY(ctx, hipMemcpyAsync(mv_out, d_mv, n * 2, hipMemcpyDeviceToHost, ctx->stream));
    HIP_TRY(ctx, hipMemcpyAsync(has_coef_out, d_has, n, hipMemcpyDeviceToHost, ctx->stream));
    HIP_TRY(ctx, hipStreamSynchronize(ctx->stream));
    return PFV_OK;
}

PFV_API int pfv_decode_plane_into(pfv_ctx *ctx, const int16_t *coef, int bw, int bh, const int32_t q[64],
                                  uint8_t *target)
{
    if (!ctx) return fail(nullptr, PFV_ERR_BAD_ARG, "null ctx");
    if (!coef || !target || bw <= 0 || bh <= 0) return fail(ctx, PFV_ERR_BAD_ARG, "pfv_decode_plane_into: bad argument");
    HIP_TRY(ctx, hipSetDevice(ctx->device));
    FrameGeom g = plane_geom(bw * 16, bh * 16, 0);
    const int32_t *tabs[1] = {q};
    int rc = upload_qtabs(ctx, tabs, 1, true);
    if (rc) return rc;
    size_t n = (size_t)bw * bh, coef_bytes = n * 512, pad_bytes = (size_t)g.pad_frame_bytes;
    void *d_coef, *d_out;
    if ((rc = ensure_scratch(ctx, 1, coef_bytes, &d_coef))) return rc;
    if ((rc = ensure_scratch(ctx, 5, pad_bytes, &d_out))) return rc;
    HIP_TRY(ctx, hipMemcpyAsync(d_coef, coef, coef_bytes, hipMemcpyHostToDevice, ctx->stream));
    launch_dec_iframe(ctx, use_small_grid(ctx->opt_lane_mapping, g), g, (const int16_t *)d_coef, (uint8_t *)d_out, ctx->qtab_dev, nullptr);
    if ((rc = launch_check(ctx, "k_dec_iframe"))) return rc;
    HIP_TRY(ctx, hipMemcpyAsync(target, d_out, pad_bytes, hipMemcpyDeviceToHost, ctx->stream));
    HIP_TRY(ctx, hipStreamSynchronize(ctx->stream));
    return PFV_OK;
}

PFV_API int pfv_decode_plane_delta(pfv_ctx *ctx, const int8_t *mv, const uint8_t *has_coef, const int16_t *coef,
                                   int bw, int bh, const int32_t q[64], const uint8_t *ref, uint8_t *out)
{
    if (!ctx) return fail(nullptr, PFV_ERR_BAD_ARG, "null ctx");
    if (!mv || !has_coef || !coef || !ref || !out || bw <= 0 || bh <= 0)
        return fail(ctx, PFV_ERR_BAD_ARG, "pfv_decode_plane_delta: bad argument");
    HIP_TRY(ctx, hipSetDevice(ctx->device));
    FrameGeom g = plane_geom(bw * 16, bh * 16, 0);
    const int32_t *tabs[1] = {q};
    int rc = upload_qtabs(ctx, tabs, 1, true);
    if (rc) return rc;
    size_t n = (size_t)bw * bh, coef_bytes = n * 512, pad_bytes = (size_t)g.pad_frame_bytes;
    void *d_coef, *d_ref, *d_mv, *d_has, *d_out;
    if ((rc = ensure_scratch(ctx, 1, coef_bytes, &d_coef))) return rc;
    if ((rc = ensure_scratch(ctx, 2, pad_bytes, &d_ref))) return rc;
    if ((rc = ensure_scratch(ctx, 3, n * 2, &d_mv))) return rc;
    if ((rc = ensure_scratch(ctx, 4, n, &d_has))) return rc;
    if ((rc = ensure_scratch(ctx, 5, pad_bytes, &d_out))) return rc;
    HIP_TRY(ctx, hipMemcpyAsync(d_coef, coef, coef_bytes, hipMemcpyHostToDevice, ctx->stream));
    HIP_TRY(ctx, hipMemcpyAsync(d_ref, ref, pad_bytes, hipMemcpyHostToDevice, ctx->stream));
    HIP_TRY(ctx, hipMemcpyAsync(d_mv, mv, n * 2, hipMemcpyHostToDevice, ctx->stream));
    HIP_TRY(ctx, hipMemcpyAsync(d_has, has_coef, n, hipMemcpyHostToDevice, ctx->stream));
    HIP_TRY(ctx, hipMemsetAsync(ctx->flag_dev, 0, sizeof(int), ctx->stream));
    launch_dec_pframe(ctx, use_small_grid(ctx->opt_lane_mapping, g), g, (const int8_t *)d_mv, (const uint8_t *)d_has, (const int16_t *)d_coef, (const uint8_t *)d_ref,
                      (uint8_t *)d_out, ctx->qtab_dev, ctx->flag_dev, nullptr);
    if ((rc = launch_check(ctx, "k_dec_pframe"))) return rc;
    int flag = 0;
    HIP_TRY(ctx, hipMemcpyAsync(&flag, ctx->flag_dev, sizeof(int), hipMemcpyDeviceToHost, ctx->stream));
    HIP_TRY(ctx, hipStreamSynchronize(ctx->stream));
    if (flag) return fail(ctx, PFV_ERR_BAD_MV, "motion vector points outside the reference plane (src/common.rs:258-259)");
    HIP_TRY(ctx, hipMemcpy(out, d_out, pad_bytes, hipMemcpyDeviceToHost));
    return PFV_OK;
}

PFV_API int pfv_decode_plane_delta_into(pfv_ctx *ctx, const int8_t *mv, const uint8_t *has_coef,
                                        const int16_t *coef, int bw, int bh, const int32_t q[64],
                                        uint8_t *ref_and_target)
{
    return pfv_decode_plane_delta(ctx, mv, has_coef, coef, bw, bh, q, ref_and_target, ref_and_target);
}

PFV_API int pfv_blit_dev(pfv_ctx *ctx, uint8_t *dst, int dst_w, int dst_h, const uint8_t *src, int src_w, int src_h,
                         int dx, int dy, int sx, int sy, int sw, int sh)
{
    if (!ctx) return fail(nullptr, PFV_ERR_BAD_ARG, "null ctx");
    if (!dst || !src || sw < 0 || sh < 0 || dx < 0 || dy < 0 || sx < 0 || sy < 0 || dx + sw > dst_w || dy + sh > dst_h ||
        sx + sw > src_w || sy + sh > src_h)
        return fail(ctx, PFV_ERR_BAD_ARG, "pfv_blit_dev: rectangle outside a plane (the reference panics on slice bounds)");
    if (sw == 0 || sh == 0) return PFV_OK;
    HIP_TRY(ctx, hipSetDevice(ctx->device));
    long n = (long)sw * sh;
    int blocks = (int)((n + kThreads - 1) / kThreads);
    if (blocks > 4096) blocks = 4096;
    hipLaunchKernelGGL(k_blit, dim3(blocks), dim3(kThreads), 0, ctx->stream, dst, dst_w, src, src_w, dx, dy, sx, sy, sw, sh);
    return launch_check(ctx, "k_blit");
}

PFV_API int pfv_reduce_dev(pfv_ctx *ctx, uint8_t *dst, const uint8_t *src, int src_w, int src_h)
{
    if (!ctx) return fail(nullptr, PFV_ERR_BAD_ARG, "null ctx");
    if (!dst || !src || src_w < 0 || src_h < 0) return fail(ctx, PFV_ERR_BAD_ARG, "pfv_reduce_dev: bad argument");
    long n = (long)(src_w / 2) * (src_h / 2);
    if (n == 0) return PFV_OK;
    HIP_TRY(ctx, hipSetDevice(ctx->device));
    int blocks = (int)((n + kThreads - 1) / kThreads);
    if (blocks > 4096) blocks = 4096;
    hipLaunchKernelGGL(k_reduce2x, dim3(blocks), dim3(kThreads), 0, ctx->stream, dst, src, src_w, src_h);
    return launch_check(ctx, "k_reduce2x");
}
PFV_API int pfv_double_dev(pfv_ctx *ctx, uint8_t *dst, const uint8_t *src, int src_w, int src_h)
{
    if (!ctx) return fail(nullptr, PFV_ERR_BAD_ARG, "null ctx");
    if (!dst || !src || src_w < 0 || src_h < 0) return fail(ctx, PFV_ERR_BAD_ARG, "pfv_double_dev: bad argument");
    long n = (long)src_w * src_h * 4;
    if (n == 0) return PFV_OK;
    HIP_TRY(ctx, hipSetDevice(ctx->device));
    int blocks = (int)((n + kThreads - 1) / kThreads);
// ... 125 lines not shown
```

pretty-fast-video_amd/csrc/pfv_sessions.hip:

```cpp
static int init_padded(pfv_ctx *ctx, const FrameGeom &g, uint8_t *buf)
{
    dim3 grid(64, 3, g.n_streams);
    hipLaunchKernelGGL(k_init_padded, grid, dim3(kThreads), 0, ctx->stream, g, buf);
    return launch_check(ctx, "k_init_padded");
}

struct XformNorms {
    double F1[8];
    double Iabs[8][8];
    signed char fsign[64];
    signed char isign[64];
};
static const XformNorms &xform_norms()
{
    static const XformNorms t = [] {
        XformNorms n{};
        for (int k = 0; k < 8; k++) {
            int f[8] = {0, 0, 0, 0, 0, 0, 0, 0}, i8[8] = {0, 0, 0, 0, 0, 0, 0, 0};
            f[k] = i8[k] = 1 << 20;
            fdct8(f);
            idct8(i8);
            for (int u = 0; u < 8; u++) {
                n.F1[u] += fabs((double)f[u]) / (1 << 20);
                n.Iabs[u][k] = fabs((double)i8[u]) / (1 << 20);
// ... 1 lines not shown
                n.isign[u * 8 + k] = (signed char)(i8[u] < 0 ? -1 : 1);
            }
        }
        return n;
    }();
    return t;
}
static double enc_max_coef(const int32_t q[64], double amplitude, int i)
{
    const XformNorms &n = xform_norms();
    const double M = amplitude * n.F1[i >> 3] * n.F1[i & 7];
    return floor(floor(M * H_SCALE[i] / 65536.0) / (double)q[i]);
}
static bool enc_float_exact(const int32_t q[64], double amplitude)
{
    const XformNorms &nm = xform_norms();
    double D[8][8], worst = 0;
    for (int i = 0; i < 64; i++) {
        const int u = i >> 3, v = i & 7, z = H_INV_ZIGZAG[i];
        const double M = amplitude * nm.F1[u] * nm.F1[v];
        const double c = enc_max_coef(q, amplitude, i);
        D[u][v] = c * (double)H_SCALE[z] * (double)q[z];
        worst = std::max(worst, std::max(M, D[u][v]));
    }
    double col[8][8];
    for (int u = 0; u < 8; u++)
        for (int v = 0; v < 8; v++) {
            double a = 16;
            for (int k = 0; k < 8; k++) a += nm.Iabs[u][k] * D[k][v];
            col[u][v] = a;
            worst = std::max(worst, a);
        }
    for (int u = 0; u < 8; u++)
        for (int v = 0; v < 8; v++) {
            double a = 16;
            for (int k = 0; k < 8; k++) a += col[u][k] * nm.Iabs[v][k];
            worst = std::max(worst, a);
        }
    return worst < 8388608.0;
}

constexpr int kMaxRungs = 11;
struct pfv_enc_session {
    pfv_ctx *ctx = nullptr;
    int width = 0, height = 0, n_streams = 0;
    FrameGeom geom;
    QTab *qtab_dev = nullptr;
    int n_rungs = 1, rung = 0;
    int qualities[kMaxRungs] = {0};
    float px_err[kMaxRungs] = {0.0f};
    bool flt = false;
    int tile_compaction = 1;
    int lane_mapping = PFV_LANES_AUTO;
    uint8_t *prev[2] = {nullptr, nullptr};
    int cur = 0;
    int win_first = 0, win_count = 0;
    size_t in_stride = 0;
    uint8_t *st_frames = nullptr;
    int16_t *st_coef = nullptr;
    int8_t *st_mv = nullptr;
    uint8_t *st_has = nullptr;
    uint32_t *q_map = nullptr;
    uint64_t *q_sse = nullptr;
    uint64_t *report_host = nullptr;
    uint32_t *probe_acc = nullptr;
    uint32_t *probe_sizes = nullptr;
    bool ent_on = false;
    uint32_t ent_cap = 0;
    EntBufs ent{};
    std::vector<void *> ent_allocs;
    std::vector<uint32_t> ent_sizes;
    uint8_t *ent_packed = nullptr;
    uint32_t *ent_offsets_dev = nullptr;
    size_t ent_packed_cap = 0;
    hipStream_t ent_stream = nullptr;
    hipEvent_t ev_encoded = nullptr;
    hipEvent_t ev_packed[2] = {nullptr, nullptr};
    int ev_cur = 0;
    bool ev_prev_valid = false;
};

struct pfv_dec_session {
    pfv_ctx *ctx = nullptr;
    int width = 0, height = 0, n_streams = 0, n_qtables = 0;
    FrameGeom geom;
    QTab *qtab_dev = nullptr;
    uint8_t *fb[2] = {nullptr, nullptr};
    int lane_mapping = PFV_LANES_AUTO;
    int cur = 0;
    int *flag_dev = nullptr;
    std::vector<int> flags_host;
    uint8_t *frames_out = nullptr;
    size_t out_stride = 0;
    int win_first = 0, win_count = 0;
    int16_t *st_coef = nullptr;
    int8_t *st_mv = nullptr;
    uint8_t *st_has = nullptr;
    uint8_t *st_frames = nullptr;
    uint32_t *st_idx = nullptr;
    int16_t *st_val = nullptr;
    size_t st_sparse_cap = 0;
    uint32_t *q_map = nullptr;
};
static int enc_report_enqueue(pfv_enc_session *s);

extern "C" {

PFV_API int pfv_enc_session_create_ladder(pfv_ctx *ctx, int width, int height, const int *qualities, int n_rungs, int n_streams,
                                          pfv_enc_session **out)
{
    if (!ctx || !out) return fail(ctx, PFV_ERR_BAD_ARG, "pfv_enc_session_create: bad argument");
    *out = nullptr;
    if (width <= 0 || height <= 0 || (width & 1) || (height & 1) || width > 65535 || height > 65535)
        return fail(ctx, PFV_ERR_BAD_ARG, "width/height must be even (src/frame.rs:13) and fit u16 (src/enc.rs:195-196)");
    if (!qualities || n_rungs < 1 || n_rungs > kMaxRungs) return fail(ctx, PFV_ERR_BAD_ARG, "a quality ladder has 1..11 rungs");
    for (int r = 0; r < n_rungs; r++) {
        if (qualities[r] < 0 || qualities[r] > 10) return fail(ctx, PFV_ERR_BAD_ARG, "quality must be in 0..10 (src/enc.rs:38)");
        if (r && qualities[r] <= qualities[r - 1]) return fail(ctx, PFV_ERR_BAD_ARG, "the qualities of a ladder must be strictly ascending");
    }
    if (n_streams <= 0) return fail(ctx, PFV_ERR_BAD_ARG, "n_streams must be positive");
    HIP_TRY(ctx, hipSetDevice(ctx->device));
    pfv_enc_session *s = new pfv_enc_session();
    s->ctx = ctx; s->width = width; s->height = height; s->n_streams = n_streams;
    s->win_count = n_streams;
    s->geom = frame_geom(width, height, n_streams);
    s->n_rungs = n_rungs;
    std::vector<QTab> tabs((size_t)4 * n_rungs);
    bool exact = true;
    for (int r = 0; r < n_rungs; r++) {
        int32_t q[4][64];
        s->qualities[r] = qualities[r];
        pfv_qtables_from_quality(qualities[r], q[0], q[1], q[2], q[3], &s->px_err[r]);
        for (int i = 0; i < 4; i++) {
            int rc = make_qtab(ctx, q[i], &tabs[(size_t)4 * r + i]);
            if (rc) { delete s; return rc; }
        }
        exact = exact && enc_float_exact(q[0], 128.0 * 256.0) && enc_float_exact(q[1], 128.0 * 256.0) && enc_float_exact(q[2], 127.0 * 256.0) &&
                enc_float_exact(q[3], 127.0 * 256.0);
    }
    s->tile_compaction = ctx->opt_tile_compaction;
    s->lane_mapping = ctx->opt_lane_mapping;
    s->flt = ctx->opt_enc_transform != PFV_ENC_TRANSFORM_INT && exact;
    size_t pad_bytes = (size_t)s->geom.pad_frame_bytes * n_streams;
    hipError_t e = hipMalloc((void **)&s->qtab_dev, tabs.size() * sizeof(QTab));
    if (e == hipSuccess) e = hipMemcpy(s->qtab_dev, tabs.data(), tabs.size() * sizeof(QTab), hipMemcpyHostToDevice);
    if (e == hipSuccess) e = hipMalloc((void **)&s->prev[0], pad_bytes);
    if (e == hipSuccess) e = hipMalloc((void **)&s->prev[1], pad_bytes);
    if (e != hipSuccess) {
        int rc = hip_fail(ctx, e, "pfv_enc_session_create");
        pfv_enc_session_destroy(s);
        return rc;
    }
    int rc = init_padded(ctx, s->geom, s->prev[0]);
    if (!rc) rc = init_padded(ctx, s->geom, s->prev[1]);
    if (rc) { pfv_enc_session_destroy(s); return rc; }
    *out = s;
    return PFV_OK;
}
PFV_API int pfv_enc_session_create(pfv_ctx *ctx, int width, int height, int quality, int n_streams,
                                   pfv_enc_session **out)
{
    return pfv_enc_session_create_ladder(ctx, width, height, &quality, 1, n_streams, out);
}
PFV_API int pfv_enc_session_set_rung(pfv_enc_session *s, int rung)
{
    if (!s) return fail(nullptr, PFV_ERR_BAD_ARG, "null session");
    if (rung < 0 || rung >= s->n_rungs) return fail(s->ctx, PFV_ERR_BAD_ARG, "pfv_enc_session_set_rung: rung outside the ladder");
    s->rung = rung;
    return PFV_OK;
}
PFV_API int pfv_enc_session_rung(pfv_enc_session *s) { return s ? s->rung : PFV_ERR_BAD_ARG; }
PFV_API int pfv_enc_session_rungs(pfv_enc_session *s) { return s ? s->n_rungs : PFV_ERR_BAD_ARG; }

PFV_API void pfv_enc_session_destroy(pfv_enc_session *s)
{
    if (!s) return;
    (void)hipSetDevice(s->ctx->device);
    (void)hipStreamSynchronize(s->ctx->stream);
    void *bufs[] = {s->qtab_dev, s->prev[0], s->prev[1], s->st_frames, s->st_coef, s->st_mv, s->st_has, s->q_map, s->q_sse, s->probe_acc, s->probe_sizes};
    for (void *b : bufs)
        if (b) (void)hipFree(b);
    for (void *b : s->ent_allocs)
        if (b) (void)hipFree(b);
    if (s->ent_packed) (void)hipFree(s->ent_packed);
    if (s->ent_offsets_dev) (void)hipFree(s->ent_offsets_dev);
    if (s->ent_stream) {
        (void)hipStreamSynchronize(s->ent_stream);
        (void)hipEventDestroy(s->ev_encoded);
        (void)hipEventDestroy(s->ev_packed[0]);
        (void)hipEventDestroy(s->ev_packed[1]);
        (void)hipStreamDestroy(s->ent_stream);
    }
    delete s;
}

static FrameGeom enc_win_geom(const pfv_enc_session *s, int count, const uint8_t *frames_win)
{
    FrameGeom g = s->geom;
    g.n_streams = count;
    if (s->in_stride) {
        g.src_frame_bytes = (long)s->in_stride;
        if (s->in_stride % 16)
            for (int i = 0; i < 3; i++) g.p[i].fast_src = 0;
    }
    return with_base_alignment(g, frames_win);
}
static int enc_launch(pfv_enc_session *s, bool pframe, int first, int count, const uint8_t *frames_dev, int8_t *mv_dev, uint8_t *has_dev,
                      int16_t *coef_dev, const uint8_t *const *slots_dev = nullptr)
{
    pfv_ctx *ctx = s->ctx;
    const size_t stride = s->in_stride ? s->in_stride : (size_t)s->geom.src_frame_bytes;
    const uint8_t *src = frames_dev + (size_t)first * stride;
    const size_t mb0 = (size_t)first * (size_t)s->geom.mbs_per_frame, pad0 = (size_t)first * (size_t)s->geom.pad_frame_bytes;
    FrameGeom g = enc_win_geom(s, count, src);
    if (slots_dev) g.src_slots = slots_dev + first;
    const int nxt = s->cur ^ 1;
    const QTab *rung_tabs = s->qtab_dev + 4 * s->rung;
    if (pframe) {
        const float min_err = s->px_err[s->rung] * s->px_err[s->rung] * 256.0f;
        launch_enc_pframe(ctx, s->flt, use_small_grid(s->lane_mapping, g), s->tile_compaction, g, src, s->prev[s->cur] + pad0, mv_dev + mb0 * 2,
                          has_dev + mb0, coef_dev + mb0 * 256, s->prev[nxt] + pad0, rung_tabs + 2, min_err);
        return launch_check(ctx, "k_enc_pframe");
    }
    launch_enc_iframe(ctx, s->flt, use_small_grid(s->lane_mapping, g), g, src, coef_dev + mb0 * 256, s->prev[nxt] + pad0, rung_tabs + 0);
    return launch_check(ctx, "k_enc_iframe");
}

PFV_API int pfv_enc_session_set_window(pfv_enc_session *s, int first, int count)
{
    if (!s) return fail(nullptr, PFV_ERR_BAD_ARG, "null session");
    if (first < 0 || count <= 0 || first > s->n_streams - count) return fail(s->ctx, PFV_ERR_BAD_ARG, "pfv_enc_session_set_window: window outside [0, n_streams)");
    s->win_first = first; s->win_count = count;
    return PFV_OK;
}
PFV_API int pfv_enc_session_set_frame_stride(pfv_enc_session *s, size_t bytes)
{
    if (!s) return fail(nullptr, PFV_ERR_BAD_ARG, "null session");
    if (bytes && bytes < (size_t)s->geom.src_frame_bytes) return fail(s->ctx, PFV_ERR_BAD_ARG, "pfv_enc_session_set_frame_stride: stride below pfv_frame_bytes");
    s->in_stride = bytes;
    return PFV_OK;
}
static bool enc_full_window(const pfv_enc_session *s) { return s->win_first == 0 && s->win_count == s->n_streams && s->in_stride == 0; }

PFV_API int pfv_enc_iframe_dev(pfv_enc_session *s, const uint8_t *frames_dev, int16_t *coef_dev)
{
    if (!s) return fail(nullptr, PFV_ERR_BAD_ARG, "null session");
    pfv_ctx *ctx = s->ctx;
    if (!frames_dev || !coef_dev) return fail(ctx, PFV_ERR_BAD_ARG, "pfv_enc_iframe_dev: null buffer");
    HIP_TRY(ctx, hipSetDevice(ctx->device));
    int rc = enc_launch(s, false, s->win_first, s->win_count, frames_dev, nullptr, nullptr, coef_dev);
    if (rc) return rc;
    s->cur ^= 1;
    return PFV_OK;
}

PFV_API int pfv_enc_pframe_dev(pfv_enc_session *s, const uint8_t *frames_dev, int8_t *mv_dev, uint8_t *has_coef_dev,
                               int16_t *coef_dev)
{
    if (!s) return fail(nullptr, PFV_ERR_BAD_ARG, "null session");
    pfv_ctx *ctx = s->ctx;
    if (!frames_dev || !mv_dev || !has_coef_dev || !coef_dev) return fail(ctx, PFV_ERR_BAD_ARG, "pfv_enc_pframe_dev: null buffer");
    HIP_TRY(ctx, hipSetDevice(ctx->device));
    int rc = enc_launch(s, true, s->win_first, s->win_count, frames_dev, mv_dev, has_coef_dev, coef_dev);
    if (rc) return rc;
    s->cur ^= 1;
    return PFV_OK;
}

static int enc_staging(pfv_enc_session *s)
{
    pfv_ctx *ctx = s->ctx;
    if (s->st_frames) return PFV_OK;
    size_t n = (size_t)s->geom.mbs_per_frame * s->n_streams;
    HIP_TRY(ctx, hipMalloc((void **)&s->st_frames, (size_t)s->geom.src_frame_bytes * s->n_streams));
    HIP_TRY(ctx, hipMalloc((void **)&s->st_coef, n * 512));
    HIP_TRY(ctx, hipMalloc((void **)&s->st_mv, n * 2));
    HIP_TRY(ctx, hipMalloc((void **)&s->st_has, n));
// ... 236 lines not shown
        s->ent_packed_cap = want;
    }
    if (!s->ent_offsets_dev) HIP_TRY(ctx, hipMalloc((void **)&s->ent_offsets_dev, (size_t)S * 4));
    HIP_TRY(ctx, hipMemcpyAsync(s->ent_offsets_dev, off.data(), (size_t)S * 4, hipMemcpyHostToDevice, st));
    EntFrame f{};
    f.n_streams = S;
    f.cap_bytes = s->ent_cap;
    f.ones16 = 0x00010001u;
    hipLaunchKernelGGL(k_ent_gather, dim3(32, (unsigned)S), dim3(kEntThreads), 0, st, f, s->ent, s->ent_offsets_dev, s->ent_packed);
    if ((rc = launch_check(ctx, "k_ent_gather"))) return rc;
    HIP_TRY(ctx, hipMemcpyAsync(out, s->ent_packed, total, hipMemcpyDeviceToHost, st));
    HIP_TRY(ctx, hipStreamSynchronize(st));
    return PFV_OK;
}

PFV_API const uint8_t *pfv_enc_payload_dev(pfv_enc_session *s, int stream)
{
    if (!s || !s->ent_on || stream < 0 || stream >= s->n_streams) return nullptr;
    return s->ent.payload + (size_t)stream * s->ent_cap;
}
PFV_API size_t pfv_enc_payload_capacity(pfv_enc_session *s) { return s && s->ent_on ? s->ent_cap : 0; }
PFV_API int pfv_enc_payload_fetch(pfv_enc_session *s, int stream, uint8_t *out, size_t nbytes)
{
    if (!s || !out) return fail(s ? s->ctx : nullptr, PFV_ERR_BAD_ARG, "pfv_enc_payload_fetch: bad argument");
    pfv_ctx *ctx = s->ctx;
    if (!s->ent_on) return fail(ctx, PFV_ERR_STATE, "call pfv_enc_entropy_enable first");
    if (stream < 0 || stream >= s->n_streams || nbytes > s->ent_cap) return fail(ctx, PFV_ERR_BAD_ARG, "pfv_enc_payload_fetch: out of range");
    hipStream_t st = s->ent_stream ? s->ent_stream : ctx->stream;
    if (nbytes) HIP_TRY(ctx, hipMemcpyAsync(out, s->ent.payload + (size_t)stream * s->ent_cap, nbytes, hipMemcpyDeviceToHost, st));
    HIP_TRY(ctx, hipStreamSynchronize(st));
    return PFV_OK;
}

PFV_API int pfv_dec_session_create(pfv_ctx *ctx, int width, int height, const int32_t *qtables, int n_qtables,
                                   int n_streams, pfv_dec_session **out)
{
    if (!ctx || !out) return fail(ctx, PFV_ERR_BAD_ARG, "pfv_dec_session_create: bad argument");
    *out = nullptr;
    if (width <= 0 || height <= 0 || (width & 1) || (height & 1) || width > 65535 || height > 65535)
        return fail(ctx, PFV_ERR_BAD_ARG, "width/height must be even (src/frame.rs:13) and fit u16");
    if ((!qtables && n_qtables > 0) || n_qtables < 0 || n_qtables > 65535 || n_streams <= 0)
        return fail(ctx, PFV_ERR_BAD_ARG, "pfv_dec_session_create: bad q-table set or stream count");
    HIP_TRY(ctx, hipSetDevice(ctx->device));
    const int n_dev = std::min(n_qtables, 256);
    std::vector<QTab> tabs((size_t)std::max(n_dev, 1));
    for (int i = 0; i < n_dev; i++) {
        int rc = make_qtab(ctx, qtables + (size_t)i * 64, &tabs[i], true);
        if (rc) return rc;
    }
    pfv_dec_session *s = new pfv_dec_session();
    s->ctx = ctx; s->width = width; s->height = height; s->n_streams = n_streams; s->n_qtables = n_qtables;
    s->win_count = n_streams;
    s->lane_mapping = ctx->opt_lane_mapping;
    s->geom = frame_geom(width, height, n_streams);
    size_t pad_bytes = (size_t)s->geom.pad_frame_bytes * n_streams;
    hipError_t e = hipMalloc((void **)&s->qtab_dev, tabs.size() * sizeof(QTab));
    if (e == hipSuccess) e = hipMemcpy(s->qtab_dev, tabs.data(), tabs.size() * sizeof(QTab), hipMemcpyHostToDevice);
    if (e == hipSuccess) e = hipMalloc((void **)&s->fb[0], pad_bytes);
    if (e == hipSuccess) e = hipMalloc((void **)&s->fb[1], pad_bytes);
    if (e == hipSuccess) e = hipMalloc((void **)&s->flag_dev, (size_t)n_streams * sizeof(int));
    if (e == hipSuccess) e = hipMemset(s->flag_dev, 0, (size_t)n_streams * sizeof(int));
    if (e != hipSuccess) {
        int rc = hip_fail(ctx, e, "pfv_dec_session_create");
        pfv_dec_session_destroy(s);
        return rc;
    }
    int rc = init_padded(ctx, s->geom, s->fb[0]);
    if (!rc) rc = init_padded(ctx, s->geom, s->fb[1]);
    if (rc) { pfv_dec_session_destroy(s); return rc; }
    *out = s;
    return PFV_OK;
}

PFV_API void pfv_dec_session_destroy(pfv_dec_session *s)
{
    if (!s) return;
    (void)hipSetDevice(s->ctx->device);
    (void)hipStreamSynchronize(s->ctx->stream);
    void *bufs[] = {s->qtab_dev, s->fb[0], s->fb[1], s->flag_dev, s->st_coef, s->st_mv, s->st_has, s->st_frames, s->st_idx, s->st_val, s->q_map};
    for (void *b : bufs)
        if (b) (void)hipFree(b);
    delete s;
}

PFV_API int pfv_dec_set_output_dev(pfv_dec_session *s, uint8_t *frames_out_dev)
{
    if (!s) return fail(nullptr, PFV_ERR_BAD_ARG, "null session");
    s->frames_out = frames_out_dev;
    s->out_stride = 0;
    return PFV_OK;
}
PFV_API int pfv_dec_set_output_strided_dev(pfv_dec_session *s, uint8_t *frames_out_dev, size_t stride_bytes)
{
    if (!s) return fail(nullptr, PFV_ERR_BAD_ARG, "null session");
    if (stride_bytes && stride_bytes < (size_t)s->geom.src_frame_bytes)
        return fail(s->ctx, PFV_ERR_BAD_ARG, "pfv_dec_set_output_strided_dev: stride below pfv_frame_bytes (the slots' frames would overlap)");
    s->frames_out = frames_out_dev;
    s->out_stride = stride_bytes;
    return PFV_OK;
}
PFV_API int pfv_dec_session_set_window(pfv_dec_session *s, int first, int count)
{
    if (!s) return fail(nullptr, PFV_ERR_BAD_ARG, "null session");
    if (first < 0 || count <= 0 || first > s->n_streams - count) return fail(s->ctx, PFV_ERR_BAD_ARG, "pfv_dec_session_set_window: window outside [0, n_streams)");
    s->win_first = first; s->win_count = count;
    return PFV_OK;
}
static bool dec_full_window(const pfv_dec_session *s) { return s->win_first == 0 && s->win_count == s->n_streams && s->out_stride == 0; }

static FrameGeom dec_out_geom(const pfv_dec_session *s, FrameGeom g, const uint8_t *out_base)
{
    if (s->out_stride) {
        g.src_frame_bytes = (long)s->out_stride;
        if (s->out_stride % 16)
            for (int i = 0; i < 3; i++) g.p[i].fast_src = 0;
    }
    return with_base_alignment(g, out_base);
}
static bool fused_output_ok(const pfv_dec_session *s)
{
    if (!s->frames_out) return false;
    FrameGeom g = dec_out_geom(s, s->geom, s->frames_out);
    return g.p[0].fast_src && g.p[1].fast_src && g.p[2].fast_src;
}

static int dec_geom(pfv_dec_session *s, const uint8_t qidx[3], FrameGeom *g)
{
    if (!qidx) return fail(s->ctx, PFV_ERR_BAD_ARG, "qidx is null");
    *g = s->geom;
    for (int i = 0; i < 3; i++) {
        if (qidx[i] >= s->n_qtables)
            return fail(s->ctx, PFV_ERR_FORMAT, "q-table index out of range (the reference panics: src/dec.rs:249-251)");
        g->p[i].qsel = qidx[i];
    }
    return PFV_OK;
}
static int dec_crop_win(pfv_dec_session *s, int first, int count, uint8_t *frames_out_dev, size_t out_stride);

static int dec_launch(pfv_dec_session *s, bool pframe, int first, int count, const int8_t *mv_dev, const uint8_t *has_dev, const DecCoefs &coefs,
                      const uint8_t qidx[3])
{
    pfv_ctx *ctx = s->ctx;
    FrameGeom g;
    int rc = dec_geom(s, qidx, &g);
    if (rc) return rc;
    const size_t ostride = s->out_stride ? s->out_stride : (size_t)s->geom.src_frame_bytes;
    const size_t mb0 = (size_t)first * (size_t)s->geom.mbs_per_frame, pad0 = (size_t)first * (size_t)s->geom.pad_frame_bytes;
    const bool fused = fused_output_ok(s);
    uint8_t *crop = fused ? s->frames_out + (size_t)first * ostride : nullptr;
    g = dec_out_geom(s, g, s->frames_out);
    g.n_streams = count;
    const int nxt = s->cur ^ 1;
    if (pframe) {
        launch_dec_pframe(ctx, use_small_grid(s->lane_mapping, g), g, mv_dev + mb0 * 2, has_dev + mb0, coefs.shifted((size_t)first, (size_t)s->geom.mbs_per_frame),
                          s->fb[s->cur] + pad0, s->fb[nxt] + pad0, s->qtab_dev, s->flag_dev + first, crop);
        rc = launch_check(ctx, "k_dec_pframe");
    } else {
        launch_dec_iframe(ctx, use_small_grid(s->lane_mapping, g), g, coefs.shifted((size_t)first, (size_t)s->geom.mbs_per_frame), s->fb[nxt] + pad0, s->qtab_dev, crop);
        rc = launch_check(ctx, "k_dec_iframe");
    }
    return rc;
}

}
static int dec_step(pfv_dec_session *s, bool pframe, const int8_t *mv_dev, const uint8_t *has_coef_dev, const DecCoefs &coefs, const uint8_t qidx[3])
{
    pfv_ctx *ctx = s->ctx;
    HIP_TRY(ctx, hipSetDevice(ctx->device));
    int rc = dec_launch(s, pframe, s->win_first, s->win_count, mv_dev, has_coef_dev, coefs, qidx);
    if (rc) return rc;
    s->cur ^= 1;
    if (s->frames_out && !fused_output_ok(s)) return dec_crop_win(s, s->win_first, s->win_count, s->frames_out, s->out_stride);
    return PFV_OK;
}
extern "C" {

PFV_API int pfv_dec_iframe_dev(pfv_dec_session *s, const int16_t *coef_dev, const uint8_t qidx[3])
{
    if (!s) return fail(nullptr, PFV_ERR_BAD_ARG, "null session");
    if (!coef_dev) return fail(s->ctx, PFV_ERR_BAD_ARG, "pfv_dec_iframe_dev: null buffer");
    return dec_step(s, false, nullptr, nullptr, coef_dev, qidx);
}

PFV_API int pfv_dec_pframe_dev(pfv_dec_session *s, const int8_t *mv_dev, const uint8_t *has_coef_dev,
                               const int16_t *coef_dev, const uint8_t qidx[3])
{
    if (!s) return fail(nullptr, PFV_ERR_BAD_ARG, "null session");
    if (!mv_dev || !has_coef_dev || !coef_dev) return fail(s->ctx, PFV_ERR_BAD_ARG, "pfv_dec_pframe_dev: null buffer");
    return dec_step(s, true, mv_dev, has_coef_dev, coef_dev, qidx);
}

PFV_API int pfv_dec_iframe_lists_dev(pfv_dec_session *s, const uint32_t *const *entries_dev, const uint32_t *counts_dev, const uint8_t qidx[3])
{
    if (!s) return fail(nullptr, PFV_ERR_BAD_ARG, "null session");
    if (!entries_dev || !counts_dev) return fail(s->ctx, PFV_ERR_BAD_ARG, "pfv_dec_iframe_lists_dev: null buffer");
    return dec_step(s, false, nullptr, nullptr, DecCoefs(entries_dev, counts_dev), qidx);
}
PFV_API int pfv_dec_pframe_lists_dev(pfv_dec_session *s, const int8_t *mv_dev, const uint8_t *has_coef_dev, const uint32_t *const *entries_dev,
                                     const uint32_t *counts_dev, const uint8_t qidx[3])
{
    if (!s) return fail(nullptr, PFV_ERR_BAD_ARG, "null session");
    if (!mv_dev || !has_coef_dev || !entries_dev || !counts_dev) return fail(s->ctx, PFV_ERR_BAD_ARG, "pfv_dec_pframe_lists_dev: null buffer");
    return dec_step(s, true, mv_dev, has_coef_dev, DecCoefs(entries_dev, counts_dev), qidx);
}
PFV_API int pfv_coef_lists_from_dense(const int16_t *coef, const uint8_t *has_coef, int total_blocks, uint32_t *entries_out, size_t cap, uint32_t *counts_out,
                                      size_t *n_out)
{
    if (!coef || !entries_out || !counts_out || !n_out || total_blocks <= 0) return fail(nullptr, PFV_ERR_BAD_ARG, "pfv_coef_lists_from_dense: bad argument");
    ListSink sink{entries_out, cap, counts_out, (size_t)total_blocks};
    bool full = false;
    for (size_t b = 0; b < (size_t)total_blocks && !full; b++) {
// ... 185 lines not shown
```

Before: 1.456 billion.

## Pair partial chroma strips of U and V planes into shared waves

Adds a chroma-pairing mode, on by default. The leftover partial strip at the right edge of each U row is merged with the matching V strip so that one wave processes both, and the remaining V strips are remapped. This cuts the number of underfilled waves in the encode I/P-frame and decode I-frame kernels. It also adds a minimum waves-per-EU attribute to the I-frame encoder, and it adds templated index-remapping paths that carry extra branching and register cost.

```diff
diff --git a/include/pfv_hip_ext.h b/include/pfv_hip_ext.h
--- a/include/pfv_hip_ext.h
+++ b/include/pfv_hip_ext.h
@@ -14,7 +14,7 @@
 
 typedef enum pfv_option {
     PFV_OPT_ENC_TRANSFORM = 1, PFV_OPT_TILE_COMPACTION = 2, PFV_OPT_LANE_MAPPING = 3, PFV_OPT_ENTROPY_DECODE = 4,
-    PFV_OPT_ENTDEC_LANE_BITS = 5, PFV_OPT_ENTDEC_LAUNCHES = 6, PFV_OPT_ENTDEC_INNER_ROUNDS = 7
+    PFV_OPT_ENTDEC_LANE_BITS = 5, PFV_OPT_ENTDEC_LAUNCHES = 6, PFV_OPT_ENTDEC_INNER_ROUNDS = 7, PFV_OPT_CHROMA_PAIRING = 8
 } pfv_option;
 enum { PFV_ENTROPY_DECODE_AUTO = 0, PFV_ENTROPY_DECODE_HOST = 1, PFV_ENTROPY_DECODE_DEVICE = 2 };
 enum { PFV_LANES_AUTO = 0, PFV_LANES_PER_MB_8 = 1, PFV_LANES_PER_MB_16 = 2 };
diff --git a/pretty-fast-video_amd/_lib.py b/pretty-fast-video_amd/_lib.py
--- a/pretty-fast-video_amd/_lib.py
+++ b/pretty-fast-video_amd/_lib.py
@@ -25,6 +25,7 @@
 PFV_LANES_AUTO, PFV_LANES_PER_MB_8, PFV_LANES_PER_MB_16 = 0, 1, 2
 PFV_OPT_ENTROPY_DECODE = 4
 PFV_OPT_ENTDEC_LANE_BITS, PFV_OPT_ENTDEC_LAUNCHES, PFV_OPT_ENTDEC_INNER_ROUNDS = 5, 6, 7
+PFV_OPT_CHROMA_PAIRING = 8
 PFV_ENTROPY_DECODE_AUTO, PFV_ENTROPY_DECODE_HOST, PFV_ENTROPY_DECODE_DEVICE = 0, 1, 2
 PFV_ENC_TRANSFORM_AUTO, PFV_ENC_TRANSFORM_INT = 0, 1
 PFV_FRAME_PACKED, PFV_FRAME_PADDED = 0, 1
diff --git a/pretty-fast-video_amd/csrc/pfv_context.hip b/pretty-fast-video_amd/csrc/pfv_context.hip
--- a/pretty-fast-video_amd/csrc/pfv_context.hip
+++ b/pretty-fast-video_amd/csrc/pfv_context.hip
@@ -12,6 +12,7 @@
     int opt_enc_transform = PFV_ENC_TRANSFORM_AUTO;
     int opt_tile_compaction = 1;
     int opt_lane_mapping = PFV_LANES_AUTO;
+    int opt_chroma_pairing = 1;
     int opt_entropy_decode = PFV_ENTROPY_DECODE_AUTO;
     int opt_entdec_lane_bits = (int)kEdSubBits, opt_entdec_launches = 3, opt_entdec_inner = kEdInner;
     std::vector<struct pfv_comm *> comms;
@@ -80,6 +81,10 @@
         if (value != PFV_LANES_AUTO && value != PFV_LANES_PER_MB_8 && value != PFV_LANES_PER_MB_16) return fail(ctx, PFV_ERR_BAD_ARG, "PFV_OPT_LANE_MAPPING: unknown value");
         ctx->opt_lane_mapping = value;
         return PFV_OK;
+    case PFV_OPT_CHROMA_PAIRING:
+        if (value != 0 && value != 1) return fail(ctx, PFV_ERR_BAD_ARG, "PFV_OPT_CHROMA_PAIRING: 0 or 1");
+        ctx->opt_chroma_pairing = value;
+        return PFV_OK;
     case PFV_OPT_ENTROPY_DECODE:
         if (value != PFV_ENTROPY_DECODE_AUTO && value != PFV_ENTROPY_DECODE_HOST && value != PFV_ENTROPY_DECODE_DEVICE) return fail(ctx, PFV_ERR_BAD_ARG, "PFV_OPT_ENTROPY_DECODE: unknown value");
         ctx->opt_entropy_decode = value;
@@ -111,6 +116,7 @@
     case PFV_OPT_ENTDEC_LANE_BITS: *value = ctx->opt_entdec_lane_bits; return PFV_OK;
     case PFV_OPT_ENTDEC_LAUNCHES: *value = ctx->opt_entdec_launches; return PFV_OK;
     case PFV_OPT_ENTDEC_INNER_ROUNDS: *value = ctx->opt_entdec_inner; return PFV_OK;
+    case PFV_OPT_CHROMA_PAIRING: *value = ctx->opt_chroma_pairing; return PFV_OK;
     default: return fail(ctx, PFV_ERR_BAD_ARG, "pfv_ctx_get_option: unknown option");
     }
 }
diff --git a/pretty-fast-video_amd/csrc/pfv_device.h b/pretty-fast-video_amd/csrc/pfv_device.h
--- a/pretty-fast-video_amd/csrc/pfv_device.h
+++ b/pretty-fast-video_amd/csrc/pfv_device.h
@@ -3,7 +3,9 @@
 
 #ifdef PFV_HIPEMU
 #define PFV_WAVES_PER_EU(n)
+#define PFV_MIN_WAVES_PER_EU(n)
 #else
+#define PFV_MIN_WAVES_PER_EU(n) __attribute__((amdgpu_waves_per_eu(n)))
 #define PFV_WAVES_PER_EU(n) __attribute__((amdgpu_waves_per_eu(n, n)))
 #endif
 
@@ -44,6 +46,7 @@
     int tiles_per_frame;
     int mbs_per_frame;
     int n_streams;
+    int pair_k;
     long src_frame_bytes;
     long pad_frame_bytes;
     const uint8_t *const *src_slots;
diff --git a/pretty-fast-video_amd/csrc/pfv_gop.hip b/pretty-fast-video_amd/csrc/pfv_gop.hip
--- a/pretty-fast-video_amd/csrc/pfv_gop.hip
+++ b/pretty-fast-video_amd/csrc/pfv_gop.hip
@@ -105,6 +105,7 @@
     k->opt_enc_transform = u->opt_enc_transform;
     k->opt_tile_compaction = u->opt_tile_compaction;
     k->opt_lane_mapping = u->opt_lane_mapping;
+    k->opt_chroma_pairing = u->opt_chroma_pairing;
 }
 
 static int gop_enc_submit(pfv_gop_encoder *e, GopEncBatch &B)
diff --git a/pretty-fast-video_amd/csrc/pfv_kernels.hip b/pretty-fast-video_amd/csrc/pfv_kernels.hip
--- a/pretty-fast-video_amd/csrc/pfv_kernels.hip
+++ b/pretty-fast-video_amd/csrc/pfv_kernels.hip
@@ -102,7 +102,10 @@
     int x0, y0;
     int n_mb;
     int mb_first;
+    int pk;
 };
+__device__ __forceinline__ long pair_dpad(const PlaneGeom &p) { return (long)p.pw * (p.ph - 1); }
+__device__ __forceinline__ int pair_dmb(const PlaneGeom &p) { return p.bw * (p.bh - 1); }
 
 __device__ __forceinline__ int plane_of(const FrameGeom &g, int idx, bool tiles)
 {
@@ -112,10 +115,22 @@
 __device__ __forceinline__ void finish_strip(const FrameGeom &g, StripPos &s)
 {
     const PlaneGeom &p = g.p[s.plane];
-    s.x0 = s.sx * (kStripMB * 16);
+    int xmb = s.sx * kStripMB, row_mbs = p.bw;
+    s.pk = 0;
+    if (g.pair_k && s.plane == 1) {
+        const int full = p.bw / kStripMB;
+        if (s.sx == full) {
+            s.pk = g.pair_k;
+            row_mbs = 2 * p.bw;
+        } else if (s.sx > full) {
+            s.plane = 2;
+            xmb -= p.bw;
+        }
+    }
+    s.x0 = xmb * 16;
     s.y0 = s.by * 16;
-    s.n_mb = min(kStripMB, p.bw - s.sx * kStripMB);
-    s.mb_first = p.mb0 + s.by * p.bw + s.sx * kStripMB;
+    s.n_mb = min(kStripMB, row_mbs - xmb);
+    s.mb_first = g.p[s.plane].mb0 + s.by * p.bw + xmb;
 }
 __device__ __forceinline__ StripPos locate_strip(const FrameGeom &g, int gstrip)
 {
@@ -261,12 +276,12 @@
     __builtin_nontemporal_store(v.z, &p->z); __builtin_nontemporal_store(v.w, &p->w);
 }
 
-__device__ __forceinline__ uint4 load_src16(const uint8_t *plane, const PlaneGeom &p, int x, int y)
+__device__ __forceinline__ uint4 load_src16(const uint8_t *plane, const PlaneGeom &p, int x, int y, int yoff = 0)
 {
     unsigned fill = (unsigned)p.clear * 0x01010101u;
     uint4 val = make_uint4(fill, fill, fill, fill);
     if (y < p.h && x < p.w) {
-        const uint8_t *src = plane + (long)y * p.w + x;
+        const uint8_t *src = plane + (long)(y + yoff) * p.w + x;
         if (p.fast_src && x + 16 <= p.w) {
             val = *reinterpret_cast<const uint4 *>(src);
         } else {
@@ -297,9 +312,16 @@
                       __builtin_amdgcn_alignbyte(d3, d2, sh), __builtin_amdgcn_alignbyte(d4, d3, sh));
 }
 
-__device__ __forceinline__ void store_cropped16(uint8_t *plane, const PlaneGeom &p, int x, int y, const uint4 &val)
-{
-    if (y < p.h && x < p.w) st_stream(reinterpret_cast<uint4 *>(plane + (long)y * p.w + x), val);
+__device__ __forceinline__ void store_cropped16(uint8_t *plane, const PlaneGeom &p, int x, int y, const uint4 &val, int yoff = 0)
+{
+    if (y < p.h && x < p.w) st_stream(reinterpret_cast<uint4 *>(plane + (long)(y + yoff) * p.w + x), val);
+}
+
+template <bool PAIR>
+__device__ __forceinline__ void store_cropped_strip(uint8_t *plane, const PlaneGeom &p, const StripPos &sp, int m, int y, const uint4 &val)
+{
+    const bool v = PAIR && m >= sp.pk;
+    store_cropped16(plane, p, sp.x0 + m * 16 - (v ? p.pw : 0), y, val, v ? p.h : 0);
 }
 
 typedef __attribute__((address_space(3))) void lds_void_t;
@@ -324,6 +346,37 @@
         buf[j] = make_uint4(0, 0, 0, 0);
         if (mb < n_mb) buf[j] = ld_stream(&reinterpret_cast<const uint4 *>(coef_mb0)[mb * 32 + h * 16 + (ch & 15)]);
     }
+}
+__device__ __forceinline__ void store_coef_half_pair(const int *stage, int16_t *coef_mb0, int n_mb, int lane, int h, int pk, int dmb)
+{
+#pragma unroll
+    for (int j = 0; j < 2; j++) {
+        int ch = j * 64 + lane;
+        int mb = ch >> 4;
+        if (mb < n_mb) st_stream(&reinterpret_cast<uint4 *>(coef_mb0)[(mb + (mb >= pk ? dmb : 0)) * 32 + h * 16 + (ch & 15)], reinterpret_cast<const uint4 *>(stage)[stage_chunk(ch)]);
+    }
+}
+__device__ __forceinline__ void fetch_coef_half_pair(uint4 (&buf)[2], const int16_t *coef_mb0, int n_mb, int lane, int h, int pk, int dmb)
+{
+#pragma unroll
+    for (int j = 0; j < 2; j++) {
+        int ch = j * 64 + lane;
+        int mb = ch >> 4;
+        buf[j] = make_uint4(0, 0, 0, 0);
+        if (mb < n_mb) buf[j] = ld_stream(&reinterpret_cast<const uint4 *>(coef_mb0)[(mb + (mb >= pk ? dmb : 0)) * 32 + h * 16 + (ch & 15)]);
+    }
+}
+template <bool PAIR>
+__device__ __forceinline__ void store_coef_strip(const int *stage, int16_t *coef_mb0, const StripPos &sp, const PlaneGeom &p, int lane, int h)
+{
+    if (PAIR) store_coef_half_pair(stage, coef_mb0, sp.n_mb, lane, h, sp.pk, pair_dmb(p));
+    else store_coef_half(stage, coef_mb0, sp.n_mb, lane, h);
+}
+template <bool PAIR>
+__device__ __forceinline__ void fetch_coef_strip(uint4 (&buf)[2], const int16_t *coef_mb0, const StripPos &sp, const PlaneGeom &p, int lane, int h)
+{
+    if (PAIR) fetch_coef_half_pair(buf, coef_mb0, sp.n_mb, lane, h, sp.pk, pair_dmb(p));
+    else fetch_coef_half(buf, coef_mb0, sp.n_mb, lane, h);
 }
 __device__ __forceinline__ void store_coef_quads(const int *stage, int16_t *coef_mb0, int n_mb, int lane, int half_strip)
 {
@@ -596,14 +649,76 @@
     }
 }
 
+template <bool FLT, int LPM, bool PAIR>
+__device__ __forceinline__ void enc_iframe_strip(const FrameGeom &g, const StripPos &sp, int half_strip, const uint8_t *src,
+                                                 int16_t *coef, uint8_t *recon, const QTab *qtabs, float qmagic,
+                                                 int *xw, int *qtab, int lane)
+{
+    constexpr int kPasses = LPM == 8 ? 2 : 1;
+    const PlaneGeom &p = g.p[sp.plane];
+    const int slot = lane >> 3, i = lane & 7;
+    const int m = LPM == 8 ? slot : half_strip * 4 + (slot >> 1);
+    const bool vslot = PAIR && m >= sp.pk;
+
+    fill_qtable<true, FLT>(qtab, qtabs + p.qsel, lane);
+    const uint8_t *plane = frame_src(g, src, sp.stream) + p.src_off;
+    uint4 rows[kPasses];
+#pragma unroll
+    for (int pass = 0; pass < kPasses; pass++)
+        rows[pass] = load_src16(plane, p, sp.x0 + m * 16 - (vslot ? p.pw : 0), sp.y0 + i + 8 * (LPM == 8 ? pass : (slot & 1)), vslot ? p.h : 0);
+
+    wave_lds_sync();
+    const LaneQ lq{qtab, i};
+    uint8_t *dst = recon ? recon + (long)sp.stream * g.pad_frame_bytes + p.pad_off + (long)(sp.y0 + i) * p.pw + sp.x0 + m * 16
+                         : nullptr;
+    if (PAIR && recon && vslot) dst += pair_dpad(p);
+    int16_t *coef_mb0 = coef + ((long)sp.stream * g.mbs_per_frame + sp.mb_first) * 256;
+#pragma unroll
+    for (int pass = 0; pass < kPasses; pass++) {
+        const int h = LPM == 8 ? pass : (slot & 1);
+        if (FLT) {
+            f2 x[8];
+            unpack_row_f(rows[pass], x);
+#pragma unroll
+            for (int k = 0; k < 8; k++) x[k] = x[k] * f2s(256.0f) - f2s(32768.0f);
+            forward_half_f(x, xw, slot, i, lq, qmagic);
+            if (LPM == 8) store_coef_strip<PAIR>(xw, coef_mb0, sp, p, lane, h);
+            else store_coef_quads(xw, coef_mb0, sp.n_mb, lane, half_strip);
+            wave_lds_sync();
+            if (recon) {
+                inverse_half_f<true>(x, xw, slot, i, lq);
+                if (m < sp.n_mb) *reinterpret_cast<uint4 *>(dst + (long)(8 * h) * p.pw) = pack_row_f(x);
+            }
+        } else {
+            int v[2][8];
+            unpack_row(rows[pass], v);
+#pragma unroll
+            for (int s = 0; s < 2; s++) {
+#pragma unroll
+                for (int k = 0; k < 8; k++) v[s][k] = (int)((unsigned)(v[s][k] - 128) << 8);
+            }
+            forward_half(v, xw, slot, i, lq, true);
+            if (LPM == 8) store_coef_strip<PAIR>(xw, coef_mb0, sp, p, lane, h);
+            else store_coef_quads(xw, coef_mb0, sp.n_mb, lane, half_strip);
+            wave_lds_sync();
+            if (recon) {
+                inverse_half(v, xw, slot, i, lq);
+#pragma unroll
+                for (int s = 0; s < 2; s++)
+#pragma unroll
+                    for (int k = 0; k < 8; k++) v[s][k] = min(max(v[s][k] + 128, 0), 255);
+                if (m < sp.n_mb) *reinterpret_cast<uint4 *>(dst + (long)(8 * h) * p.pw) = pack_row(v);
+            }
+        }
+    }
+}
 template <bool FLT, int LPM = 8>
-__global__ __launch_bounds__(kThreads) void k_enc_iframe(FrameGeom g, const uint8_t *__restrict__ src,
+__global__ __launch_bounds__(kThreads) PFV_MIN_WAVES_PER_EU((LPM == 8 && FLT) ? 7 : 8) void k_enc_iframe(FrameGeom g, const uint8_t *__restrict__ src,
                                                           int16_t *__restrict__ coef, uint8_t *__restrict__ recon,
                                                           const QTab *__restrict__ qtabs, float qmagic)
 {
     __shared__ __attribute__((aligned(16))) int xchg[kStripsPerWG][kXchgDwords];
     __shared__ __attribute__((aligned(16))) int qtab_lds[kStripsPerWG][kQTabDwords];
-    constexpr int kPasses = LPM == 8 ? 2 : 1;
 
     const int lane = threadIdx.x & 63, wave = __builtin_amdgcn_readfirstlane((int)(threadIdx.x >> 6));
     const int gw = xcd_remap((int)blockIdx.x, (int)gridDim.x) * kStripsPerWG + wave;
@@ -611,59 +726,10 @@
     if (gstrip >= g.strips_per_frame * g.n_streams) return;
     const StripPos sp = locate_strip(g, gstrip);
     if (half_strip * 4 >= sp.n_mb) return;
-    const PlaneGeom &p = g.p[sp.plane];
-    const int slot = lane >> 3, i = lane & 7;
-    const int m = LPM == 8 ? slot : half_strip * 4 + (slot >> 1);
-    int *xw = xchg[wave];
-
-    fill_qtable<true, FLT>(qtab_lds[wave], qtabs + p.qsel, lane);
-    const uint8_t *plane = frame_src(g, src, sp.stream) + p.src_off;
-    uint4 rows[kPasses];
-#pragma unroll
-    for (int pass = 0; pass < kPasses; pass++) rows[pass] = load_src16(plane, p, sp.x0 + m * 16, sp.y0 + i + 8 * (LPM == 8 ? pass : (slot & 1)));
-
-    wave_lds_sync();
-    const LaneQ lq{qtab_lds[wave], i};
-    int16_t *coef_mb0 = coef + ((long)sp.stream * g.mbs_per_frame + sp.mb_first) * 256;
-    uint8_t *dst = recon ? recon + (long)sp.stream * g.pad_frame_bytes + p.pad_off + (long)(sp.y0 + i) * p.pw + sp.x0 + m * 16
-                         : nullptr;
-#pragma unroll
-    for (int pass = 0; pass < kPasses; pass++) {
-        const int h = LPM == 8 ? pass : (slot & 1);
-        if (FLT) {
-            f2 x[8];
-            unpack_row_f(rows[pass], x);
-#pragma unroll
-            for (int k = 0; k < 8; k++) x[k] = x[k] * f2s(256.0f) - f2s(32768.0f);
-            forward_half_f(x, xw, slot, i, lq, qmagic);
-            if (LPM == 8) store_coef_half(xw, coef_mb0, sp.n_mb, lane, h);
-            else store_coef_quads(xw, coef_mb0, sp.n_mb, lane, half_strip);
-            wave_lds_sync();
-            if (recon) {
-                inverse_half_f<true>(x, xw, slot, i, lq);
-                if (m < sp.n_mb) *reinterpret_cast<uint4 *>(dst + (long)(8 * h) * p.pw) = pack_row_f(x);
-            }
-        } else {
-            int v[2][8];
-            unpack_row(rows[pass], v);
-#pragma unroll
-            for (int s = 0; s < 2; s++) {
-#pragma unroll
-                for (int k = 0; k < 8; k++) v[s][k] = (int)((unsigned)(v[s][k] - 128) << 8);
-            }
-            forward_half(v, xw, slot, i, lq, true);
-            if (LPM == 8) store_coef_half(xw, coef_mb0, sp.n_mb, lane, h);
-            else store_coef_quads(xw, coef_mb0, sp.n_mb, lane, half_strip);
-            wave_lds_sync();
-            if (recon) {
-                inverse_half(v, xw, slot, i, lq);
-#pragma unroll
-                for (int s = 0; s < 2; s++)
-#pragma unroll
-                    for (int k = 0; k < 8; k++) v[s][k] = min(max(v[s][k] + 128, 0), 255);
-                if (m < sp.n_mb) *reinterpret_cast<uint4 *>(dst + (long)(8 * h) * p.pw) = pack_row(v);
-            }
-        }
+    if (LPM == 8 && sp.pk) {
+        enc_iframe_strip<FLT, LPM, LPM == 8>(g, sp, half_strip, src, coef, recon, qtabs, qmagic, xchg[wave], qtab_lds[wave], lane);
+    } else {
+        enc_iframe_strip<FLT, LPM, false>(g, sp, half_strip, src, coef, recon, qtabs, qmagic, xchg[wave], qtab_lds[wave], lane);
     }
 }
 
@@ -904,10 +970,24 @@
     return t;
 }
 
+template <bool PAIR = false>
 __device__ __forceinline__ void issue_window(const PlaneGeom &p, const uint8_t *refp, const TilePos &t, uint8_t *winbuf, int wave,
                                              int lane)
 {
     const int q0 = win_first_issue(wave), q1 = win_first_issue(wave + 1);
+    if (PAIR) {
+        const int pk = t.sp.pk;
+#pragma unroll 5
+        for (int q = q0; q < q1; q++) {
+            const int c = q * 64 + lane;
+            const int row = c / kWinChunksPerRow, col = c - row * kWinChunksPerRow;
+            const bool v = col > pk;
+            const int y = min(max(t.winy0 + row, 0), p.ph - 1) + (v ? p.ph : 0);
+            const int x = min(max(v ? (col - 1 - pk) * 16 : t.winx0 + col * 16, 0), p.pw - 16);
+            __builtin_amdgcn_global_load_lds((gbl_cvoid_t *)(refp + (long)y * p.pw + x), (lds_void_t *)(winbuf + c * 16), 16, 0, 0);
+        }
+        return;
+    }
 #pragma unroll 5
     for (int q = q0; q < q1; q++) {
         const int c = q * 64 + lane;
@@ -923,7 +1003,7 @@
     uint4 patch[2];
 };
 
-template <bool DPPRED = false>
+template <bool DPPRED = false, bool PAIR = false>
 __device__ __forceinline__ void penc_search(const FrameGeom &g, const TilePos &tp, const uint8_t *win, int *red, const uint4 (&rows)[2], int lane,
                                             float min_err, int neg2, SearchOut &so)
 {
@@ -931,8 +1011,9 @@
     const PlaneGeom &p = g.p[sp.plane];
     const int m = lane >> 3, i = lane & 7;
     const bool mb_valid = m < sp.n_mb;
-    const int mbx = sp.x0 + m * 16, mby = sp.y0;
-    const int wcol0 = mbx - tp.winx0;
+    const int mbx = sp.x0 + m * 16 - (PAIR && m >= sp.pk ? p.pw : 0);
+    const int mby = sp.y0;
+    const int wcol0 = 16 + m * 16;
     const int wrow0 = mby - tp.winy0 + i;
 
     unsigned s2 = 0;
@@ -949,7 +1030,7 @@
     st.cx = 0; st.cy = 0; st.err = 0;
     const SearchLane sl = make_search_lane(red, m, i, neg2);
     const bool interior = sp.x0 >= 16 && sp.x0 + kStripMB * 16 + 16 <= p.pw && sp.y0 >= 16 && sp.y0 + 32 <= p.ph;
-    if (interior) {
+    if (!PAIR && interior) {
         search_level<8, true, false, DPPRED>(win, wrow0, wcol0, rows[0], rows[1], a2, mbx, mby, p.pw, p.ph, st, sl);
         KMARK(3);
         search_level<4, false, false, DPPRED>(win, wrow0, wcol0, rows[0], rows[1], a2, mbx, mby, p.pw, p.ph, st, sl);
@@ -1054,7 +1135,7 @@
     }
 }
 
-template <bool FLT>
+template <bool FLT, bool PAIR = false>
 __device__ __forceinline__ void penc_transform(const FrameGeom &g, const TilePos &tp, const SearchOut &so, const uint4 (&rows)[2], int *xw,
                                                int lane, int16_t *__restrict__ coef, uint8_t *__restrict__ recon, const int *qtab_lds, float qmagic)
 {
@@ -1065,22 +1146,23 @@
     const int mbx = sp.x0 + m * 16;
     int16_t *coef_mb0 = coef + ((long)sp.stream * g.mbs_per_frame + sp.mb_first) * 256;
     uint8_t *dst = recon ? recon + (long)sp.stream * g.pad_frame_bytes + p.pad_off + (long)(sp.y0 + i) * p.pw + mbx : nullptr;
+    if (PAIR && recon && m >= sp.pk) dst += pair_dpad(p);
 
     if (__any(coded)) {
         const LaneQ lq{qtab_lds, i};
 #pragma unroll
         for (int h = 0; h < 2; h++) {
             const uint4 o = penc_half<FLT>(coded ? rows[h] : so.patch[h], so.patch[h], xw, m, i, lq, qmagic, recon != nullptr,
-                                           [&]() { store_coef_half(xw, coef_mb0, sp.n_mb, lane, h); });
+                                           [&]() { store_coef_strip<PAIR>(xw, coef_mb0, sp, p, lane, h); });
             if (h == 0) KMARK(9);
             if (recon && mb_valid) *reinterpret_cast<uint4 *>(dst + (long)(8 * h) * p.pw) = o;
         }
     } else if (mb_valid) {
-        penc_store_skipped(coef_mb0 + m * 256, dst, p.pw, i, so.patch);
-    }
-}
-
-template <bool FLT>
+        penc_store_skipped(coef_mb0 + (m + (PAIR && m >= sp.pk ? pair_dmb(p) : 0)) * 256, dst, p.pw, i, so.patch);
+    }
+}
+
+template <bool FLT, bool PAIR = false>
 __device__ __forceinline__ void penc_transform_compact(const FrameGeom &g, const TilePos &tp, int wave, int n_coded, const int *slot_orig,
                                                        const uint4 *staged, int *xw, int lane, int16_t *__restrict__ coef,
                                                        uint8_t *__restrict__ recon, const int *qtab_lds, float qmagic)
@@ -1089,7 +1171,7 @@
     const int m = lane >> 3, i = lane & 7;
     const int slot = wave * 8 + m;
     const bool has = slot < n_coded;
-    const long tile_mb0 = (long)tp.sp.stream * g.mbs_per_frame + p.mb0 + (long)(tp.plane_ty * kStripsPerWG) * p.bw + tp.sp.sx * kStripMB;
+    const long tile_mb0 = (long)tp.sp.stream * g.mbs_per_frame + p.mb0 + (long)(tp.plane_ty * kStripsPerWG) * p.bw + (tp.sp.x0 >> 4);
     const LaneQ lq{qtab_lds, i};
     const uint4 *sl = staged + (has ? slot : 0) * 32 + i * 4;
 #pragma unroll
@@ -1102,7 +1184,7 @@
                 const int ch = j * 64 + lane, sc = wave * 8 + (ch >> 4);
                 if (sc < n_coded) {
                     const int og = slot_orig[sc];
-                    int16_t *mb = coef + (tile_mb0 + (long)(og >> 3) * p.bw + (og & 7)) * 256;
+                    int16_t *mb = coef + (PAIR ? tile_mb0 + slot_orig[kPencCompactMax + sc] : tile_mb0 + (long)(og >> 3) * p.bw + (og & 7)) * 256;
                     st_stream(&reinterpret_cast<uint4 *>(mb)[h * 16 + (ch & 15)], reinterpret_cast<const uint4 *>(xw)[stage_chunk(ch)]);
                 }
             }
@@ -1111,39 +1193,34 @@
             const int orig = slot_orig[slot];
             uint8_t *dst = recon + (long)tp.sp.stream * g.pad_frame_bytes + p.pad_off +
                            (long)((tp.plane_ty * kStripsPerWG + (orig >> 3)) * 16 + i + 8 * h) * p.pw + tp.sp.x0 + (orig & 7) * 16;
+            if (PAIR) dst += slot_orig[2 * kPencCompactMax + slot];
             *reinterpret_cast<uint4 *>(dst) = o;
         }
     }
 }
 
-template <bool FLT>
-__global__ __launch_bounds__(kThreads) PFV_WAVES_PER_EU(PFV_PENC_WAVES) void k_enc_pframe(FrameGeom g, const uint8_t *__restrict__ src,
-                                                          const uint8_t *__restrict__ ref, int8_t *__restrict__ mv_out,
-                                                          uint8_t *__restrict__ has_out, int16_t *__restrict__ coef,
-                                                          uint8_t *__restrict__ recon, const QTab *__restrict__ qtabs,
-                                                          float min_err, int neg2, float qmagic, int compact_max)
-{
-    __shared__ __attribute__((aligned(16))) uint8_t win_lds[16 + kWinAlloc];
-    __shared__ __attribute__((aligned(16))) int red_lds[kStripsPerWG][kRedDwords];
-    __shared__ __attribute__((aligned(16))) int qtab_lds[kQTabDwords];
-    uint8_t *win = win_lds + 16;
-
-    const int lane = threadIdx.x & 63, wave = __builtin_amdgcn_readfirstlane((int)(threadIdx.x >> 6));
+template <bool FLT, bool PAIR>
+__device__ __forceinline__ void penc_tile(const FrameGeom &g, const TilePos &cur, const uint8_t *src, const uint8_t *ref,
+                                          int8_t *mv_out, uint8_t *has_out, int16_t *coef,
+                                          uint8_t *recon, const QTab *qtabs, float min_err, int neg2, float qmagic,
+                                          int compact_max, uint8_t *win, int (*red_lds)[kRedDwords], int *qtab_lds, int lane, int wave)
+{
     const int m = lane >> 3, i = lane & 7;
-    const int vt = xcd_remap((int)blockIdx.x, (int)gridDim.x);
-    const TilePos cur = locate_tile(g, vt, wave);
     const PlaneGeom &p = g.p[cur.sp.plane];
     if (wave == 0) fill_qtable<true, FLT>(qtab_lds, qtabs + p.qsel, lane);
 
     KMARK(0);
     KMARK_WHERE();
-    issue_window(p, ref + (long)cur.sp.stream * g.pad_frame_bytes + p.pad_off, cur, win, wave, lane);
+    issue_window<PAIR>(p, ref + (long)cur.sp.stream * g.pad_frame_bytes + p.pad_off, cur, win, wave, lane);
     uint4 rows[2];
     rows[0] = rows[1] = make_uint4(0, 0, 0, 0);
+    const int pk = cur.sp.pk;
     if (cur.wave_valid) {
         const uint8_t *plane = frame_src(g, src, cur.sp.stream) + p.src_off;
-        rows[0] = load_src16(plane, p, cur.sp.x0 + m * 16, cur.sp.y0 + i);
-        rows[1] = load_src16(plane, p, cur.sp.x0 + m * 16, cur.sp.y0 + i + 8);
+        const bool v = PAIR && m >= pk;
+        const int x = cur.sp.x0 + m * 16 - (v ? p.pw : 0), yoff = v ? p.h : 0;
+        rows[0] = load_src16(plane, p, x, cur.sp.y0 + i, yoff);
+        rows[1] = load_src16(plane, p, x, cur.sp.y0 + i + 8, yoff);
     }
     KMARK(1);
     __syncthreads();
@@ -1151,11 +1228,11 @@
     SearchOut so;
     so.cx = so.cy = 0; so.coded = false;
     so.patch[0] = so.patch[1] = make_uint4(0, 0, 0, 0);
-    if (cur.wave_valid) penc_search(g, cur, win, red_lds[wave], rows, lane, min_err, neg2, so);
+    if (cur.wave_valid) penc_search<false, PAIR>(g, cur, win, red_lds[wave], rows, lane, min_err, neg2, so);
     KMARK(7);
     const bool mb_valid = cur.wave_valid && m < cur.sp.n_mb;
     if (i == 0 && mb_valid) {
-        const long mbi = (long)cur.sp.stream * g.mbs_per_frame + cur.sp.mb_first + m;
+        const long mbi = (long)cur.sp.stream * g.mbs_per_frame + cur.sp.mb_first + m + (PAIR && m >= pk ? pair_dmb(p) : 0);
         mv_out[mbi * 2 + 0] = (int8_t)so.cx;
         mv_out[mbi * 2 + 1] = (int8_t)so.cy;
         has_out[mbi] = so.coded ? 1 : 0;
@@ -1180,7 +1257,7 @@
     int *xw = reinterpret_cast<int *>(win + win_first_issue(wave) * 1024);
     constexpr int kCompactMax = kPencCompactMax;
     constexpr int kSlotOrigAt = kCompactMax * 128;
-    static_assert(kSlotOrigAt + kCompactMax <= kMaskAt, "staging area + slot table must fit below the strip masks");
+    static_assert(kSlotOrigAt + 3 * kCompactMax <= kMaskAt, "staging area + slot tables (place; PAIR: macroblock, byte offset) must fit below the strip masks");
     static_assert(kStripsPerWG * 8 <= 32, "one bit per macroblock of the tile");
     if (n_coded <= compact_max && ((n_coded + 7) >> 3) < strips_coded) {
         uint4 *stage4 = reinterpret_cast<uint4 *>(red_all);
@@ -1189,20 +1266,49 @@
             const int slot = __builtin_popcount(tile_mask & ((1u << place) - 1u));
             uint4 *sl = stage4 + slot * 32 + i * 4;
             sl[0] = rows[0]; sl[1] = rows[1]; sl[2] = so.patch[0]; sl[3] = so.patch[1];
-            if (i == 0) red_all[kSlotOrigAt + slot] = place;
+            if (i == 0) {
+                red_all[kSlotOrigAt + slot] = place;
+                if (PAIR) {
+                    red_all[kSlotOrigAt + kCompactMax + slot] = wave * p.bw + m + (m >= pk ? pair_dmb(p) : 0);
+                    red_all[kSlotOrigAt + 2 * kCompactMax + slot] = m >= pk ? (int)pair_dpad(p) : 0;
+                }
+            }
         } else if (mb_valid) {
             const PlaneGeom &pp = g.p[cur.sp.plane];
-            penc_store_skipped(coef + ((long)cur.sp.stream * g.mbs_per_frame + cur.sp.mb_first + m) * 256,
-                               recon ? recon + (long)cur.sp.stream * g.pad_frame_bytes + pp.pad_off + (long)(cur.sp.y0 + i) * pp.pw + cur.sp.x0 + m * 16 : nullptr,
-                               pp.pw, i, so.patch);
+            int16_t *cmb = coef + ((long)cur.sp.stream * g.mbs_per_frame + cur.sp.mb_first + m) * 256;
+            uint8_t *dst = recon ? recon + (long)cur.sp.stream * g.pad_frame_bytes + pp.pad_off + (long)(cur.sp.y0 + i) * pp.pw + cur.sp.x0 + m * 16 : nullptr;
+            if (PAIR && m >= pk) {
+                cmb += (long)pair_dmb(pp) * 256;
+                if (recon) dst += pair_dpad(pp);
+            }
+            penc_store_skipped(cmb, dst, pp.pw, i, so.patch);
         }
         __syncthreads();
         if (wave * 8 < n_coded)
-            penc_transform_compact<FLT>(g, cur, wave, n_coded, red_all + kSlotOrigAt, stage4, xw, lane, coef, recon, qtab_lds, qmagic);
+            penc_transform_compact<FLT, PAIR>(g, cur, wave, n_coded, red_all + kSlotOrigAt, stage4, xw, lane, coef, recon, qtab_lds, qmagic);
     } else if (cur.wave_valid) {
-        penc_transform<FLT>(g, cur, so, rows, xw, lane, coef, recon, qtab_lds, qmagic);
+        penc_transform<FLT, PAIR>(g, cur, so, rows, xw, lane, coef, recon, qtab_lds, qmagic);
     }
     KMARK(11);
+}
+template <bool FLT>
+__global__ __launch_bounds__(kThreads) PFV_WAVES_PER_EU(PFV_PENC_WAVES) void k_enc_pframe(FrameGeom g, const uint8_t *__restrict__ src,
+                                                          const uint8_t *__restrict__ ref, int8_t *__restrict__ mv_out,
+                                                          uint8_t *__restrict__ has_out, int16_t *__restrict__ coef,
+                                                          uint8_t *__restrict__ recon, const QTab *__restrict__ qtabs,
+                                                          float min_err, int neg2, float qmagic, int compact_max)
+{
+    __shared__ __attribute__((aligned(16))) uint8_t win_lds[16 + kWinAlloc];
+    __shared__ __attribute__((aligned(16))) int red_lds[kStripsPerWG][kRedDwords];
+    __shared__ __attribute__((aligned(16))) int qtab_lds[kQTabDwords];
+
+    const int lane = threadIdx.x & 63, wave = __builtin_amdgcn_readfirstlane((int)(threadIdx.x >> 6));
+    const TilePos cur = locate_tile(g, xcd_remap((int)blockIdx.x, (int)gridDim.x), wave);
+    if (cur.sp.pk) {
+        penc_tile<FLT, true>(g, cur, src, ref, mv_out, has_out, coef, recon, qtabs, min_err, neg2, qmagic, compact_max, win_lds + 16, red_lds, qtab_lds, lane, wave);
+    } else {
+        penc_tile<FLT, false>(g, cur, src, ref, mv_out, has_out, coef, recon, qtabs, min_err, neg2, qmagic, compact_max, win_lds + 16, red_lds, qtab_lds, lane, wave);
+    }
 }
 
 template <bool DPPRED>
@@ -1563,25 +1669,15 @@
     }
 }
 
-template <int LPM = 8, bool LISTS = false>
-__global__ __launch_bounds__(kThreads) void k_dec_iframe(FrameGeom g, const int16_t *__restrict__ coef, CoefLists cl,
-                                                          uint8_t *__restrict__ out, const QTab *__restrict__ qtabs,
-                                                          uint8_t *__restrict__ frames_out)
-{
-    __shared__ __attribute__((aligned(16))) int xchg[kStripsPerWG][kXchgDwords];
-    __shared__ __attribute__((aligned(16))) int qtab_lds[kStripsPerWG][kQTabDwords];
+template <int LPM, bool LISTS, bool PAIR>
+__device__ __forceinline__ void dec_iframe_strip(const FrameGeom &g, const StripPos &sp, int half_strip, const int16_t *coef, const CoefLists &cl,
+                                                 uint8_t *out, const QTab *qtabs, uint8_t *frames_out, int *xw,
+                                                 int *qtab, int lane)
+{
     constexpr int kPasses = LPM == 8 ? 2 : 1;
-
-    const int lane = threadIdx.x & 63, wave = __builtin_amdgcn_readfirstlane((int)(threadIdx.x >> 6));
-    const int gw = xcd_remap((int)blockIdx.x, (int)gridDim.x) * kStripsPerWG + wave;
-    const int gstrip = LPM == 8 ? gw : gw >> 1, half_strip = LPM == 8 ? 0 : gw & 1;
-    if (gstrip >= g.strips_per_frame * g.n_streams) return;
-    const StripPos sp = locate_strip(g, gstrip);
-    if (half_strip * 4 >= sp.n_mb) return;
     const PlaneGeom &p = g.p[sp.plane];
     const int slot = lane >> 3, i = lane & 7;
     const int m = LPM == 8 ? slot : half_strip * 4 + (slot >> 1);
-    int *xw = xchg[wave];
 
     const int16_t *coef_mb0 = coef + ((long)sp.stream * g.mbs_per_frame + sp.mb_first) * 256;
     uint4 cbuf[kPasses][2];
@@ -1592,15 +1688,16 @@
         const int mw = min(LPM == 8 ? slot : (slot >> 1), last);
         span = list_span(cl.entries[sp.stream], cnt[mw], cnt[mw + 1], last * (LPM == 8 ? 8 : 16), lane);
     } else if (LPM == 8) {
-        fetch_coef_half(cbuf[0], coef_mb0, sp.n_mb, lane, 0);
-        fetch_coef_half(cbuf[kPasses - 1], coef_mb0, sp.n_mb, lane, 1);
+        fetch_coef_strip<PAIR>(cbuf[0], coef_mb0, sp, p, lane, 0);
+        fetch_coef_strip<PAIR>(cbuf[kPasses - 1], coef_mb0, sp, p, lane, 1);
     } else {
         fetch_coef_quads(cbuf[0], coef_mb0, sp.n_mb, lane, half_strip);
     }
-    fill_qtable<false>(qtab_lds[wave], qtabs + p.qsel, lane);
+    fill_qtable<false>(qtab, qtabs + p.qsel, lane);
     wave_lds_sync();
-    const LaneQ lq{qtab_lds[wave], i};
+    const LaneQ lq{qtab, i};
     uint8_t *dst = out + (long)sp.stream * g.pad_frame_bytes + p.pad_off + (long)(sp.y0 + i) * p.pw + sp.x0 + m * 16;
+    if (PAIR && m >= sp.pk) dst += pair_dpad(p);
 #pragma unroll
     for (int pass = 0; pass < kPasses; pass++) {
         const int h = LPM == 8 ? pass : (slot & 1);
@@ -1618,8 +1715,28 @@
             const uint4 o = pack_row(v);
             *reinterpret_cast<uint4 *>(dst + (long)(8 * h) * p.pw) = o;
             if (frames_out)
-                store_cropped16(frames_out + (long)sp.stream * g.src_frame_bytes + p.src_off, p, sp.x0 + m * 16, sp.y0 + i + 8 * h, o);
-        }
+                store_cropped_strip<PAIR>(frames_out + (long)sp.stream * g.src_frame_bytes + p.src_off, p, sp, m, sp.y0 + i + 8 * h, o);
+        }
+    }
+}
+template <int LPM = 8, bool LISTS = false>
+__global__ __launch_bounds__(kThreads) PFV_MIN_WAVES_PER_EU((LPM == 8 && !LISTS) ? 7 : 8) void k_dec_iframe(FrameGeom g, const int16_t *__restrict__ coef, CoefLists cl,
+                                                          uint8_t *__restrict__ out, const QTab *__restrict__ qtabs,
+                                                          uint8_t *__restrict__ frames_out)
+{
+    __shared__ __attribute__((aligned(16))) int xchg[kStripsPerWG][kXchgDwords];
+    __shared__ __attribute__((aligned(16))) int qtab_lds[kStripsPerWG][kQTabDwords];
+
+    const int lane = threadIdx.x & 63, wave = __builtin_amdgcn_readfirstlane((int)(threadIdx.x >> 6));
+    const int gw = xcd_remap((int)blockIdx.x, (int)gridDim.x) * kStripsPerWG + wave;
+    const int gstrip = LPM == 8 ? gw : gw >> 1, half_strip = LPM == 8 ? 0 : gw & 1;
+    if (gstrip >= g.strips_per_frame * g.n_streams) return;
+    const StripPos sp = locate_strip(g, gstrip);
+    if (half_strip * 4 >= sp.n_mb) return;
+    if (LPM == 8 && !LISTS && sp.pk) {
+        dec_iframe_strip<LPM, LISTS, LPM == 8 && !LISTS>(g, sp, half_strip, coef, cl, out, qtabs, frames_out, xchg[wave], qtab_lds[wave], lane);
+    } else {
+        dec_iframe_strip<LPM, LISTS, false>(g, sp, half_strip, coef, cl, out, qtabs, frames_out, xchg[wave], qtab_lds[wave], lane);
     }
 }
 
diff --git a/pretty-fast-video_amd/csrc/pfv_launch.hip b/pretty-fast-video_amd/csrc/pfv_launch.hip
--- a/pretty-fast-video_amd/csrc/pfv_launch.hip
+++ b/pretty-fast-video_amd/csrc/pfv_launch.hip
@@ -100,6 +100,24 @@
     return g;
 }
 
+static FrameGeom paired_geom(FrameGeom g)
+{
+    if (g.n_planes != 3) return g;
+    const PlaneGeom &u = g.p[1], &v = g.p[2];
+    const int k = u.bw % kStripMB;
+    if (k == 0 || 2 * k > kStripMB) return g;
+    if (u.w != v.w || u.h != v.h || u.qsel != v.qsel || u.clear != v.clear || u.fast_src != v.fast_src) return g;
+    if (v.pad_off - u.pad_off != (long)u.pw * u.ph || v.src_off - u.src_off != (long)u.w * u.h || v.mb0 - u.mb0 != u.bw * u.bh) return g;
+    const int row_strips = (2 * u.bw + kStripMB - 1) / kStripMB;
+    g.pair_k = k;
+    g.p[1].strips_x = row_strips;
+    g.p[2].strip0 = g.p[1].strip0 + row_strips * u.bh;
+    g.p[2].tile0 = g.p[1].tile0 + row_strips * u.tiles_y;
+    g.strips_per_frame = g.p[2].strip0;
+    g.tiles_per_frame = g.p[2].tile0;
+    return g;
+}
+
 static inline unsigned penc_blocks(const pfv_ctx *, const FrameGeom &g)
 {
     return (unsigned)((long)g.tiles_per_frame * g.n_streams);
@@ -123,8 +141,9 @@
     long waves = 2 * (long)g.strips_per_frame * g.n_streams;
     return (unsigned)((waves + kStripsPerWG - 1) / kStripsPerWG);
 }
-static void launch_enc_iframe(pfv_ctx *ctx, bool flt, bool small, const FrameGeom &g, const uint8_t *src, int16_t *coef, uint8_t *recon, const QTab *qt)
-{
+static void launch_enc_iframe(pfv_ctx *ctx, bool flt, bool small, bool pair, const FrameGeom &g0, const uint8_t *src, int16_t *coef, uint8_t *recon, const QTab *qt)
+{
+    const FrameGeom g = pair && !small ? paired_geom(g0) : g0;
     if (small) {
         if (flt) hipLaunchKernelGGL((k_enc_iframe<true, 16>), dim3(half_strip_blocks(g)), dim3(kThreads), 0, ctx->stream, g, src, coef, recon, qt, kQuantMagic);
         else hipLaunchKernelGGL((k_enc_iframe<false, 16>), dim3(half_strip_blocks(g)), dim3(kThreads), 0, ctx->stream, g, src, coef, recon, qt, kQuantMagic);
@@ -133,10 +152,11 @@
         else hipLaunchKernelGGL((k_enc_iframe<false, 8>), dim3(strip_blocks(g)), dim3(kThreads), 0, ctx->stream, g, src, coef, recon, qt, kQuantMagic);
     }
 }
-static void launch_enc_pframe(pfv_ctx *ctx, bool flt, bool small, int compaction, const FrameGeom &g, const uint8_t *src, const uint8_t *ref, int8_t *mv,
+static void launch_enc_pframe(pfv_ctx *ctx, bool flt, bool small, bool pair, int compaction, const FrameGeom &g0, const uint8_t *src, const uint8_t *ref, int8_t *mv,
                               uint8_t *has, int16_t *coef, uint8_t *recon, const QTab *qt, float min_err)
 {
     const bool split = compaction == 2 && !small;
+    const FrameGeom g = pair && !small && !split ? paired_geom(g0) : g0;
     launch_enc_pframe_kernels(ctx->stream, flt, small, split ? kPencSplit : (compaction ? kPencCompactMax : 0), g, penc_blocks(ctx, g), src, ref, mv, has, coef, recon, qt, min_err);
     if (split) {
         const unsigned tf = (unsigned)((long)g.n_streams * tf_groups_per_frame(g));
@@ -159,8 +179,9 @@
         return c;
     }
 };
-static void launch_dec_iframe(pfv_ctx *ctx, bool small, const FrameGeom &g, const DecCoefs &c, uint8_t *out, const QTab *qt, uint8_t *frames_out)
-{
+static void launch_dec_iframe(pfv_ctx *ctx, bool small, bool pair, const FrameGeom &g0, const DecCoefs &c, uint8_t *out, const QTab *qt, uint8_t *frames_out)
+{
+    const FrameGeom g = pair && !small && !c.is_lists() ? paired_geom(g0) : g0;
     const dim3 grid(small ? half_strip_blocks(g) : strip_blocks(g)), block(kThreads);
     if (c.is_lists()) {
         if (small) hipLaunchKernelGGL((k_dec_iframe<16, true>), grid, block, 0, ctx->stream, g, c.dense, c.lists, out, qt, frames_out);
@@ -170,7 +191,7 @@
         else hipLaunchKernelGGL((k_dec_iframe<8, false>), grid, block, 0, ctx->stream, g, c.dense, c.lists, out, qt, frames_out);
     }
 }
-static void launch_dec_pframe(pfv_ctx *ctx, bool small, const FrameGeom &g, const int8_t *mv, const uint8_t *has, const DecCoefs &c, const uint8_t *ref,
+static void launch_dec_pframe(pfv_ctx *ctx, bool small, bool , const FrameGeom &g, const int8_t *mv, const uint8_t *has, const DecCoefs &c, const uint8_t *ref,
                               uint8_t *out, const QTab *qt, int *flag, uint8_t *frames_out)
 {
     const dim3 grid(small ? half_strip_blocks(g) : strip_blocks(g)), block(kThreads);
diff --git a/pretty-fast-video_amd/csrc/pfv_plane_ops.hip b/pretty-fast-video_amd/csrc/pfv_plane_ops.hip
--- a/pretty-fast-video_amd/csrc/pfv_plane_ops.hip
+++ b/pretty-fast-video_amd/csrc/pfv_plane_ops.hip
@@ -15,7 +15,7 @@
     if ((rc = ensure_scratch(ctx, 0, (size_t)w * h, &d_src))) return rc;
     if ((rc = ensure_scratch(ctx, 1, coef_bytes, &d_coef))) return rc;
     HIP_TRY(ctx, hipMemcpyAsync(d_src, px, (size_t)w * h, hipMemcpyHostToDevice, ctx->stream));
-    launch_enc_iframe(ctx, ctx->opt_enc_transform != PFV_ENC_TRANSFORM_INT, use_small_grid(ctx->opt_lane_mapping, g), g, (const uint8_t *)d_src, (int16_t *)d_coef,
+    launch_enc_iframe(ctx, ctx->opt_enc_transform != PFV_ENC_TRANSFORM_INT, use_small_grid(ctx->opt_lane_mapping, g), false, g, (const uint8_t *)d_src, (int16_t *)d_coef,
                       nullptr, ctx->qtab_dev);
     if ((rc = launch_check(ctx, "k_enc_iframe"))) return rc;
     HIP_TRY(ctx, hipMemcpyAsync(coef_out, d_coef, coef_bytes, hipMemcpyDeviceToHost, ctx->stream));
@@ -45,7 +45,7 @@
     HIP_TRY(ctx, hipMemcpyAsync(d_src, px, (size_t)w * h, hipMemcpyHostToDevice, ctx->stream));
     HIP_TRY(ctx, hipMemcpyAsync(d_ref, ref, pad_bytes, hipMemcpyHostToDevice, ctx->stream));
     float min_err = px_err * px_err * 256.0f;
-    launch_enc_pframe(ctx, ctx->opt_enc_transform != PFV_ENC_TRANSFORM_INT, use_small_grid(ctx->opt_lane_mapping, g), ctx->opt_tile_compaction, g,
+    launch_enc_pframe(ctx, ctx->opt_enc_transform != PFV_ENC_TRANSFORM_INT, use_small_grid(ctx->opt_lane_mapping, g), false, ctx->opt_tile_compaction, g,
                       (const uint8_t *)d_src, (const uint8_t *)d_ref, (int8_t *)d_mv, (uint8_t *)d_has, (int16_t *)d_coef, nullptr, ctx->qtab_dev, min_err);
     if ((rc = launch_check(ctx, "k_enc_pframe"))) return rc;
     HIP_TRY(ctx, hipMemcpyAsync(coef_out, d_coef, coef_bytes, hipMemcpyDeviceToHost, ctx->stream));
@@ -70,7 +70,7 @@
     if ((rc = ensure_scratch(ctx, 1, coef_bytes, &d_coef))) return rc;
     if ((rc = ensure_scratch(ctx, 5, pad_bytes, &d_out))) return rc;
     HIP_TRY(ctx, hipMemcpyAsync(d_coef, coef, coef_bytes, hipMemcpyHostToDevice, ctx->stream));
-    launch_dec_iframe(ctx, use_small_grid(ctx->opt_lane_mapping, g), g, (const int16_t *)d_coef, (uint8_t *)d_out, ctx->qtab_dev, nullptr);
+    launch_dec_iframe(ctx, use_small_grid(ctx->opt_lane_mapping, g), false, g, (const int16_t *)d_coef, (uint8_t *)d_out, ctx->qtab_dev, nullptr);
     if ((rc = launch_check(ctx, "k_dec_iframe"))) return rc;
     HIP_TRY(ctx, hipMemcpyAsync(target, d_out, pad_bytes, hipMemcpyDeviceToHost, ctx->stream));
     HIP_TRY(ctx, hipStreamSynchronize(ctx->stream));
@@ -100,7 +100,7 @@
     HIP_TRY(ctx, hipMemcpyAsync(d_mv, mv, n * 2, hipMemcpyHostToDevice, ctx->stream));
     HIP_TRY(ctx, hipMemcpyAsync(d_has, has_coef, n, hipMemcpyHostToDevice, ctx->stream));
     HIP_TRY(ctx, hipMemsetAsync(ctx->flag_dev, 0, sizeof(int), ctx->stream));
-    launch_dec_pframe(ctx, use_small_grid(ctx->opt_lane_mapping, g), g, (const int8_t *)d_mv, (const uint8_t *)d_has, (const int16_t *)d_coef, (const uint8_t *)d_ref,
+    launch_dec_pframe(ctx, use_small_grid(ctx->opt_lane_mapping, g), false, g, (const int8_t *)d_mv, (const uint8_t *)d_has, (const int16_t *)d_coef, (const uint8_t *)d_ref,
                       (uint8_t *)d_out, ctx->qtab_dev, ctx->flag_dev, nullptr);
     if ((rc = launch_check(ctx, "k_dec_pframe"))) return rc;
     int flag = 0;
diff --git a/pretty-fast-video_amd/csrc/pfv_sessions.hip b/pretty-fast-video_amd/csrc/pfv_sessions.hip
--- a/pretty-fast-video_amd/csrc/pfv_sessions.hip
+++ b/pretty-fast-video_amd/csrc/pfv_sessions.hip
@@ -77,6 +77,7 @@
     bool flt = false;
     int tile_compaction = 1;
     int lane_mapping = PFV_LANES_AUTO;
+    bool chroma_pairing = true;
     uint8_t *prev[2] = {nullptr, nullptr};
     int cur = 0;
     int win_first = 0, win_count = 0;
@@ -112,6 +113,7 @@
     QTab *qtab_dev = nullptr;
     uint8_t *fb[2] = {nullptr, nullptr};
     int lane_mapping = PFV_LANES_AUTO;
+    bool chroma_pairing = true;
     int cur = 0;
     int *flag_dev = nullptr;
     std::vector<int> flags_host;
@@ -165,6 +167,7 @@
     }
     s->tile_compaction = ctx->opt_tile_compaction;
     s->lane_mapping = ctx->opt_lane_mapping;
+    s->chroma_pairing = ctx->opt_chroma_pairing != 0;
     s->flt = ctx->opt_enc_transform != PFV_ENC_TRANSFORM_INT && exact;
     size_t pad_bytes = (size_t)s->geom.pad_frame_bytes * n_streams;
     hipError_t e = hipMalloc((void **)&s->qtab_dev, tabs.size() * sizeof(QTab));
@@ -243,11 +246,11 @@
     const QTab *rung_tabs = s->qtab_dev + 4 * s->rung;
     if (pframe) {
         const float min_err = s->px_err[s->rung] * s->px_err[s->rung] * 256.0f;
-        launch_enc_pframe(ctx, s->flt, use_small_grid(s->lane_mapping, g), s->tile_compaction, g, src, s->prev[s->cur] + pad0, mv_dev + mb0 * 2,
+        launch_enc_pframe(ctx, s->flt, use_small_grid(s->lane_mapping, g), s->chroma_pairing, s->tile_compaction, g, src, s->prev[s->cur] + pad0, mv_dev + mb0 * 2,
                           has_dev + mb0, coef_dev + mb0 * 256, s->prev[nxt] + pad0, rung_tabs + 2, min_err);
         return launch_check(ctx, "k_enc_pframe");
     }
-    launch_enc_iframe(ctx, s->flt, use_small_grid(s->lane_mapping, g), g, src, coef_dev + mb0 * 256, s->prev[nxt] + pad0, rung_tabs + 0);
+    launch_enc_iframe(ctx, s->flt, use_small_grid(s->lane_mapping, g), s->chroma_pairing, g, src, coef_dev + mb0 * 256, s->prev[nxt] + pad0, rung_tabs + 0);
     return launch_check(ctx, "k_enc_iframe");
 }
 
@@ -590,6 +593,7 @@
     s->ctx = ctx; s->width = width; s->height = height; s->n_streams = n_streams; s->n_qtables = n_qtables;
     s->win_count = n_streams;
     s->lane_mapping = ctx->opt_lane_mapping;
+    s->chroma_pairing = ctx->opt_chroma_pairing != 0;
     s->geom = frame_geom(width, height, n_streams);
     size_t pad_bytes = (size_t)s->geom.pad_frame_bytes * n_streams;
     hipError_t e = hipMalloc((void **)&s->qtab_dev, tabs.size() * sizeof(QTab));
@@ -690,11 +694,11 @@
     g.n_streams = count;
     const int nxt = s->cur ^ 1;
     if (pframe) {
-        launch_dec_pframe(ctx, use_small_grid(s->lane_mapping, g), g, mv_dev + mb0 * 2, has_dev + mb0, coefs.shifted((size_t)first, (size_t)s->geom.mbs_per_frame),
+        launch_dec_pframe(ctx, use_small_grid(s->lane_mapping, g), s->chroma_pairing, g, mv_dev + mb0 * 2, has_dev + mb0, coefs.shifted((size_t)first, (size_t)s->geom.mbs_per_frame),
                           s->fb[s->cur] + pad0, s->fb[nxt] + pad0, s->qtab_dev, s->flag_dev + first, crop);
         rc = launch_check(ctx, "k_dec_pframe");
     } else {
-        launch_dec_iframe(ctx, use_small_grid(s->lane_mapping, g), g, coefs.shifted((size_t)first, (size_t)s->geom.mbs_per_frame), s->fb[nxt] + pad0, s->qtab_dev, crop);
+        launch_dec_iframe(ctx, use_small_grid(s->lane_mapping, g), s->chroma_pairing, g, coefs.shifted((size_t)first, (size_t)s->geom.mbs_per_frame), s->fb[nxt] + pad0, s->qtab_dev, crop);
         rc = launch_check(ctx, "k_dec_iframe");
     }
     return rc;
```

Measured after the change: 1.456 billion (median of 2 runs). About the same (+0.0%).
